# carlobaldassi/gimp-lqr-plugin

Measured on AMD Instinct MI355X. Metric: Mseams*pixels/sec on 4K RGBA, higher is better.
Workload: dtype f32; 1 GPU; batch4k: 64 x 3840x2160 RGBA per GPU, resize to 3640x2160 (200 vertical seams each), side-switch 2; images_per_gpu=64, width=3840, height=2160, new_width=3640, new_height=2160, parallelism=images sharded i mod N, no data-path collective, streams_per_gpu=1

## Files before the change

gimp-lqr-plugin_amd/csrc/k_backtrack.hip:

```cpp
#include "lqr_common.h"
#include "lqr_kernels.h"

__device__ __forceinline__ int row_argmin(const gf32 *mrow, int w, int lr, float *s_val, int *s_idx)
{
    const int tid = threadIdx.x;
    const float INF = __int_as_float(0x7f800000);
    float bv = INF;
    int bi = -1;
    for (int base = 0; base < w; base += 16 * VPATH_THREADS) {
        f32x4 v[4];
#pragma unroll
        for (int i = 0; i < 4; i++) {
            const int x = base + 4 * (tid + VPATH_THREADS * i);
            if (x + 3 < w) v[i] = *(const GLOBAL_AS f32x4 *) (mrow + x);
            else { v[i] = (f32x4) {INF, INF, INF, INF}; for (int j = 0; j < 4; j++) if (x + j < w) v[i][j] = mrow[x + j]; }
        }
#pragma unroll
        for (int i = 0; i < 4; i++)
#pragma unroll
            for (int j = 0; j < 4; j++) {
                const int x = base + 4 * (tid + VPATH_THREADS * i) + j;
                const float f = v[i][j];
                if (x < w && (f < bv || (f == bv && lr))) { bv = f; bi = x; }
            }
    }
    auto better = [&](float v2, int i2, float v1, int i1) {
        if (i2 < 0) return false;
        if (i1 < 0) return true;
        if (v2 < v1) return true;
        if (v2 > v1) return false;
        return lr ? (i2 > i1) : (i2 < i1);
    };
    for (int o = 32; o > 0; o >>= 1) {
        const float v2 = __shfl_xor(bv, o);
        const int i2 = __shfl_xor(bi, o);
        if (better(v2, i2, bv, bi)) { bv = v2; bi = i2; }
    }
    if ((tid & 63) == 0) { s_val[tid >> 6] = bv; s_idx[tid >> 6] = bi; }
    __syncthreads();
    bv = s_val[0]; bi = s_idx[0];
#pragma unroll
    for (int k = 1; k < VPATH_THREADS / 64; k++) if (better(s_val[k], s_idx[k], bv, bi)) { bv = s_val[k]; bi = s_idx[k]; }
    const float lim = 536870912.0f;
    const bool ok = (bi >= 0) && (bv < lim || (bv == lim && lr));
    return ok ? bi : -1;
}

__device__ unsigned long long g_moved_bytes;
__device__ __forceinline__ void publish_side(const GCarver &c, int org, int acc, int w, int h, int lane, int moved_unit)
{
    for (int o = 32; o > 0; o >>= 1) acc += __shfl_xor(acc, o);
    const long long all = (long long) h * (w - 1);
    const int side = (2ll * acc < all) ? 1 : 0;
    if (lane == 0) {
        c.flags[FLAG_ORG_PREV] = org; c.flags[FLAG_SIDE] = side; c.flags[FLAG_ORG] = org + side;
        atomicAdd(&g_moved_bytes, (unsigned long long) (side ? (long long) acc : all - acc) * (unsigned long long) moved_unit);
    }
}
extern "C" int lqrhip_moved_bytes(unsigned long long *out, int reset)
{
    if (lqrhip_init() < 0) return -1;
    (void) hipDeviceSynchronize();
    if (hipMemcpyFromSymbol(out, HIP_SYMBOL(g_moved_bytes), sizeof(unsigned long long)) != hipSuccess) return -1;
    if (reset) { unsigned long long z = 0; (void) hipMemcpyToSymbol(HIP_SYMBOL(g_moved_bytes), &z, sizeof z); }
    return 0;
}

__global__ __launch_bounds__(VPATH_THREADS) void k_vpath(const DevCarver *cs, int w, int h, int stride, int lr, int delta,
                                                          int log_index, int moved_unit)
{
    const GCarver c = gview(cs[blockIdx.x]);
    const int org = c.flags[FLAG_ORG];
    __shared__ float s_val[VPATH_THREADS / 64];
    __shared__ int s_idx[VPATH_THREADS / 64];
    const int tid = threadIdx.x;

    const int xmin = row_argmin(c.m + (size_t) (h - 1) * stride, w, lr, s_val, s_idx);
    if (tid >= 64) return;
    int x = __builtin_amdgcn_readfirstlane(max(xmin, 0));

    const int lane = tid;
    gi32 *seam = c.seam_x;
    gi32 *logp = c.seam_log + (size_t) log_index * h;
    const int R = delta > 0 ? min(VP_ROWS, max(1, VP_ROWS / delta)) : VP_ROWS;
    uint32_t regs[2][VP_ROWS];
    auto window_base = [&](int cx) { return (cx - 126) & ~3; };
    auto load_chunk = [&](int b, int y_top, int xa) {
        const int xl = xa + 4 * lane;
        const bool ok = (xl >= 0) && (xl + 3 < stride);
#pragma unroll
        for (int r = 0; r < VP_ROWS; r++) {
            const int y = max(y_top - r, 0);
            regs[b][r] = ok ? *(const gu32 *) (c.least + (size_t) y * stride + xl) : 0u;
        }
    };
    int y_top = h - 1;
    int xa_cur = window_base(x);
    int acc = 0;
    if (y_top >= 1) load_chunk(0, y_top, xa_cur);
    while (y_top >= 1) {
#pragma unroll
        for (int b = 0; b < 2; b++) {
            if (y_top >= 1) {
                const int nrows = min(R, y_top);
                const int xa_next = window_base(x);
                if (y_top - nrows >= 1) load_chunk(b ^ 1, y_top - nrows, xa_next);
                int path = 0;
#pragma unroll
                for (int r = 0; r < VP_ROWS; r++) {
                    if (r < nrows) {
                        path = (lane == r) ? x : path;
                        const int o = x - xa_cur;
                        const uint32_t dw = (uint32_t) __builtin_amdgcn_readlane((int) regs[b][r], o >> 2);
                        int d = (int) (int8_t) (dw >> (8 * (o & 3)));
                        d = (d == LEAST_INVALID) ? 0 : d;
                        x += d;
                    }
                }
                if (lane < nrows) { seam[y_top - lane] = path; logp[y_top - lane] = path; acc += path; }
                xa_cur = xa_next;
                y_top -= nrows;
            }
        }
    }
    if (lane == 0) { seam[0] = x; logp[0] = x; acc += x; }
    publish_side(c, org, acc, w, h, lane, moved_unit);
}

constexpr int vp1_rows(int delta) { return delta == 1 ? 28 : delta == 2 ? 12 : delta == 3 ? 8 : 4; }
#define VP1_AHEAD 3
template <int r>
__device__ __forceinline__ void vp1_step(const int e, int &o, int &path)
{
    asm volatile("v_writelane_b32 %0, %1, %2" : "+v"(path) : "s"(o), "n"(r));
    o += __builtin_amdgcn_readlane(e, o);
}
template <int N, int... Rs>
__device__ __forceinline__ void vp1_chase(const int (&e)[N], int &o, int &path, std::integer_sequence<int, Rs...>)
{
    (vp1_step<Rs>(e[Rs], o, path), ...);
}

template <int DELTA>
__global__ __launch_bounds__(VPATH_THREADS) void k_vpath1(const DevCarver *cs, int w, int h, int stride, int lr, int log_index, int moved_unit)
{
    const GCarver c = gview(cs[blockIdx.x]);
    const int org = c.flags[FLAG_ORG];
    __shared__ float s_val[VPATH_THREADS / 64];
    __shared__ int s_idx[VPATH_THREADS / 64];
    constexpr int VP1_ROWS = vp1_rows(DELTA);
    __shared__ __attribute__((aligned(16))) int8_t s_win[VP1_ROWS * 256];
    const int tid = threadIdx.x;

    const int xmin = row_argmin(c.m + (size_t) (h - 1) * stride, w, lr, s_val, s_idx);
    if (tid >= 64) return;
    int x = __builtin_amdgcn_readfirstlane(max(xmin, 0));

    const int lane = tid;
    gi32 *seam = c.seam_x;
    gi32 *logp = c.seam_log + (size_t) log_index * h;
    constexpr int R = VP1_ROWS, NB = VP1_AHEAD + 1, RL = VP1_ROWS / 4;
    static_assert(VP1_ROWS % 4 == 0 && VP1_ROWS * DELTA <= 28 && VP1_AHEAD * VP1_ROWS * DELTA + 32 <= 120, "window margin");
    u32x4 regs[NB][RL];
    int xa[NB];
    auto window_base = [&](int cx) { return (cx - 120) & ~15; };
    auto load_chunk = [&](int b, int y_top, int cx) {
        const int base = window_base(cx);
        xa[b] = base;
        const int voff = min(max(base + 16 * (lane & 15), 0), stride - 16);
        const int rsub = (lane >> 4) * stride;
#pragma unroll
        for (int q = 0; q < RL; q++) {
            const int row = max((y_top - 4 * q) * stride - rsub, stride);
            regs[b][q] = *(const GLOBAL_AS u32x4 *) (c.least + (unsigned) (row + voff));
        }
    };
    int acc = 0;
    auto run_chunk = [&](int b, int y_top) {
        const int relbase = x - 32 - xa[b];
        int e[R];
#pragma unroll
        for (int q = 0; q < RL; q++) *(u32x4 *) (s_win + q * 1024 + lane * 16) = regs[b][q];
        __builtin_amdgcn_wave_barrier();
#pragma unroll
        for (int r = 0; r < R; r++) e[r] = s_win[r * 256 + relbase + lane];
        int e2[R / 2];
#pragma unroll
        for (int k = 0; k < R / 2; k++) e2[k] = e[2 * k] + __builtin_amdgcn_ds_bpermute((lane + e[2 * k]) << 2, e[2 * k + 1]);
        int o = 32, path = 0;
        vp1_chase<R / 2>(e2, o, path, std::make_integer_sequence<int, R / 2>{});
        const int odd = path + s_win[min(lane, R / 2 - 1) * 512 + relbase + path];
        __builtin_amdgcn_wave_barrier();
        const int pe = path + x - 32, po = odd + x - 32;
        const int nrows = min(R, y_top);
        if (2 * lane < nrows) { seam[y_top - 2 * lane] = pe; logp[y_top - 2 * lane] = pe; acc += pe; }
        if (2 * lane + 1 < nrows) { seam[y_top - 2 * lane - 1] = po; logp[y_top - 2 * lane - 1] = po; acc += po; }
        x = (nrows == R) ? x + o - 32 : __builtin_amdgcn_readlane((nrows & 1) ? po : pe, nrows >> 1);
    };
    int y_top = h - 1;
#pragma unroll
    for (int k = 0; k < VP1_AHEAD; k++) load_chunk(k, y_top - k * R, x);
    while (true) {
#pragma unroll
        for (int k = 0; k < NB; k++) {
            load_chunk((k + VP1_AHEAD) % NB, y_top - VP1_AHEAD * R, x);
            run_chunk(k, y_top);
            y_top -= R;
            if (y_top < 1) break;
        }
        if (y_top < 1) break;
    }
    if (lane == 0) { seam[0] = x; logp[0] = x; acc += x; }
    publish_side(c, org, acc, w, h, lane, moved_unit);
}


template <int DELTA>
__global__ __launch_bounds__(256) void k_vp_maps(const DevCarver *cs, int w, int h, int stride)
{
    constexpr int R = vp_chunk_rows(DELTA), RD = R * DELTA, WIN = 256 + 2 * RD, R4 = (R + 3) / 4;
    __shared__ __attribute__((aligned(4))) int8_t s_rows[R][WIN + 8];
    const GCarver c = gview(cs[blockIdx.z]);
    const int chunk = blockIdx.y, ytop = h - 1 - chunk * R, nrows = min(R, ytop);
    const int X0 = blockIdx.x * 256, base = X0 - RD, tid = threadIdx.x;
    constexpr int WD = (WIN + 3) / 4, NI = (R * WD + 255) / 256;
    uint32_t v[NI];
#pragma unroll
    for (int k = 0; k < NI; k++) {
        const int i = tid + 256 * k, r = i / WD, d = i - r * WD, col = base + 4 * d;
        v[k] = 0u;
        if (i >= nrows * WD) continue;
        if (col >= 0 && col + 3 < stride) v[k] = *(const gu32 *) (c.least + (size_t) (ytop - r) * stride + col);
        else for (int b = 0; b < 4; b++) if (col + b >= 0 && col + b < stride) v[k] |= (uint32_t) (uint8_t) c.least[(size_t) (ytop - r) * stride + col + b] << (8 * b);
    }
#pragma unroll
    for (int k = 0; k < NI; k++) {
        const int i = tid + 256 * k, r = i / WD, d = i - r * WD;
        if (i < nrows * WD) *(uint32_t *) &s_rows[r][4 * d] = v[k];
    }
    __syncthreads();
    const int x = X0 + tid;
    if (x >= w) return;
    int p = x - base;
    gu32 *path = (gu32 *) c.vp_path + (size_t) chunk * R4 * stride + x;
#pragma unroll
    for (int r4 = 0; r4 < R4; r4++) {
        uint32_t pk = 0u;
#pragma unroll
        for (int k = 0; k < 4; k++) {
            const int r = 4 * r4 + k;
            pk |= (uint32_t) (uint8_t) (int8_t) (p + base - x) << (8 * k);
            if (r < nrows) { const int d = s_rows[r < R ? r : 0][p]; p += (d == LEAST_INVALID) ? 0 : d; }
        }
        path[(size_t) r4 * stride] = pk;
    }
    c.vp_map[(size_t) chunk * stride + x] = (int8_t) (p + base - x);
}

template <int DELTA>
__global__ __launch_bounds__(VPATH_THREADS) void k_vp_solve(const DevCarver *cs, int w, int h, int stride, int lr, int log_index, int moved_unit)
{
    constexpr int R = vp_chunk_rows(DELTA), RD = R * DELTA, S = VP_STAGE, R4 = (R + 3) / 4;
    constexpr int CP = (2 * RD * S + 4 + 15 + 16) & ~15;
    const GCarver c = gview(cs[blockIdx.x]);
    const int org = c.flags[FLAG_ORG];
    __shared__ float s_val[VPATH_THREADS / 64];
    __shared__ int s_idx[VPATH_THREADS / 64];
    __shared__ __attribute__((aligned(16))) int8_t s_cone[S][CP];
    extern __shared__ int s_xs[];
    __shared__ int s_acc[VPATH_THREADS / 64];
    const int tid = threadIdx.x, lane = tid & 63;
    const int xmin = row_argmin(c.m + (size_t) (h - 1) * stride, w, lr, s_val, s_idx);
    const int nchunks = (h - 1 + R - 1) / R;
    int x = max(xmin, 0);
    for (int c0 = 0; c0 < nchunks; c0 += S) {
        const int ns = min(S, nchunks - c0);
        const int base = (x - RD * S) & ~3;
        constexpr int W16 = CP / 16, NI = (S * W16 + VPATH_THREADS - 1) / VPATH_THREADS;
        u32x4 v[NI];
#pragma unroll
        for (int k = 0; k < NI; k++) {
            const int i = tid + k * VPATH_THREADS, j = i / W16, d = i - j * W16, col = base + 16 * d;
            v[k] = (u32x4) {0u, 0u, 0u, 0u};
            if (i >= ns * W16 || col + 15 < x - RD * (j + 1) || col > x + RD * (j + 1)) continue;
            const gi8 *src = c.vp_map + (size_t) (c0 + j) * stride + col;
            if (col >= 0 && col + 15 < stride) v[k] = *(const GLOBAL_AS u32x4 *) src;
            else {
                uint32_t q4[4] = {0u, 0u, 0u, 0u};
                for (int b = 0; b < 16; b++) if (col + b >= 0 && col + b < stride) q4[b >> 2] |= (uint32_t) (uint8_t) src[b] << (8 * (b & 3));
                v[k] = (u32x4) {q4[0], q4[1], q4[2], q4[3]};
            }
        }
#pragma unroll
        for (int k = 0; k < NI; k++) {
// ... 40 lines not shown
```

gimp-lqr-plugin_amd/csrc/k_carve.hip:

```cpp
#include "lqr_common.h"
#include "lqr_kernels.h"


#ifndef CG
#define CG 4
#endif
#define CGPX (CG * 256)
struct G32 { u32x4 a[CG]; uint32_t edge; };
struct G8 { uint32_t a[CG]; uint32_t edge; };

__device__ __forceinline__ void ld_left_u32(const gu32 *row, int base, int pend, int lane, G32 &g)
{
#pragma unroll
    for (int u = 0; u < CG; u++) {
        const int x = base + u * 256 + lane * 4;
        g.a[u] = (x <= pend) ? __builtin_nontemporal_load((const GLOBAL_AS u32x4 *) (row + x)) : (u32x4) {0u, 0u, 0u, 0u};
    }
    g.edge = (lane == 63 && base + CGPX <= pend) ? row[base + CGPX] : 0u;
}
__device__ __forceinline__ void st_left_u32(gu32 *row, int base, int pv, int pend, int lane, const G32 &g)
{
#pragma unroll
    for (int u = 0; u < CG; u++) {
        const int x = base + u * 256 + lane * 4;
        const uint32_t first_next = (u < CG - 1) ? (uint32_t) __builtin_amdgcn_readlane((int) g.a[u < CG - 1 ? u + 1 : CG - 1].x, 0) : 0u;
        const uint32_t lane63 = (u < CG - 1) ? first_next : g.edge;
        const uint32_t nx = (uint32_t) __builtin_amdgcn_update_dpp((int) lane63, (int) g.a[u].x, DPP_WAVE_SHL1, 0xf, 0xf, false);
        if (x < pend) {
            u32x4 o;
            o.x = (x >= pv) ? g.a[u].y : g.a[u].x;
            o.y = (x + 1 >= pv) ? g.a[u].z : g.a[u].y;
            o.z = (x + 2 >= pv) ? g.a[u].w : g.a[u].z;
            o.w = (x + 3 >= pv) ? nx : g.a[u].w;
            __builtin_nontemporal_store(o, (GLOBAL_AS u32x4 *) (row + x));
        }
    }
}

__device__ __forceinline__ void ld_right_u32(const gu32 *row, int gbase, int pbeg, int pv, int lane, G32 &g)
{
#pragma unroll
    for (int u = 0; u < CG; u++) {
        const int x = gbase + u * 256 + lane * 4;
        g.a[u] = (x + 3 >= pbeg && x <= pv) ? __builtin_nontemporal_load((const GLOBAL_AS u32x4 *) (row + x)) : (u32x4) {0u, 0u, 0u, 0u};
    }
    g.edge = (lane == 0 && gbase - 1 >= pbeg) ? row[gbase - 1] : 0u;
}
__device__ __forceinline__ void st_right_u32(gu32 *row, int gbase, int pbeg, int pv, int lane, const G32 &g)
{
#pragma unroll
    for (int u = 0; u < CG; u++) {
        const int x = gbase + u * 256 + lane * 4;
        const uint32_t last_prev = (u > 0) ? (uint32_t) __builtin_amdgcn_readlane((int) g.a[u > 0 ? u - 1 : 0].w, 63) : 0u;
        const uint32_t lane0 = (u > 0) ? last_prev : g.edge;
        const uint32_t pw = (uint32_t) __builtin_amdgcn_update_dpp((int) lane0, (int) g.a[u].w, DPP_WAVE_SHR1, 0xf, 0xf, false);
        if (x <= pv && x + 3 > pbeg) {
            u32x4 o;
            o.x = (x > pbeg && x <= pv) ? pw : g.a[u].x;
            o.y = (x + 1 > pbeg && x + 1 <= pv) ? g.a[u].x : g.a[u].y;
            o.z = (x + 2 > pbeg && x + 2 <= pv) ? g.a[u].y : g.a[u].z;
            o.w = (x + 3 > pbeg && x + 3 <= pv) ? g.a[u].z : g.a[u].w;
            __builtin_nontemporal_store(o, (GLOBAL_AS u32x4 *) (row + x));
        }
    }
}

__device__ __forceinline__ void st_left_en(gu32 *row, int base, int x0, int pend, int lane, const G32 &g)
{
#pragma unroll
    for (int u = 0; u < CG; u++) {
        const int x = base + u * 256 + lane * 4;
        const uint32_t first_next = (u < CG - 1) ? (uint32_t) __builtin_amdgcn_readlane((int) g.a[u < CG - 1 ? u + 1 : CG - 1].x, 0) : 0u;
        const uint32_t lane63 = (u < CG - 1) ? first_next : g.edge;
        const uint32_t nx = (uint32_t) __builtin_amdgcn_update_dpp((int) lane63, (int) g.a[u].x, DPP_WAVE_SHL1, 0xf, 0xf, false);
        if (x >= x0 && x < pend) __builtin_nontemporal_store((u32x4) {g.a[u].y, g.a[u].z, g.a[u].w, nx}, (GLOBAL_AS u32x4 *) (row + x));
    }
}
__device__ __forceinline__ void st_right_en(gu32 *row, int gbase, int x0, int x1, int lane, const G32 &g)
{
#pragma unroll
    for (int u = 0; u < CG; u++) {
        const int x = gbase + u * 256 + lane * 4;
        const uint32_t last_prev = (u > 0) ? (uint32_t) __builtin_amdgcn_readlane((int) g.a[u > 0 ? u - 1 : 0].w, 63) : 0u;
        const uint32_t lane0 = (u > 0) ? last_prev : g.edge;
// ... 27 lines not shown
        const int q = xo + dx;
        if (q == vprev) dx = LEAST_INVALID;
        else dx = q - (q > vprev ? 1 : 0) - xx;
    }
    return dx;
}

__device__ __forceinline__ void ld_left_8(const gu32 *row32, int base, int pend, int lane, G8 &g)
{
#pragma unroll
    for (int u = 0; u < CG; u++) {
        const int x = base + u * 256 + lane * 4;
        g.a[u] = (x <= pend) ? __builtin_nontemporal_load(row32 + (x >> 2)) : 0u;
    }
    g.edge = (lane == 63 && base + CGPX <= pend) ? row32[(base + CGPX) >> 2] : 0u;
}
__device__ __forceinline__ void st_left_8(gu32 *row32, int base, int org, int start, int v, int vprev, int y, int wnew, int lane, const G8 &g)
{
    const int pend = org + wnew;
#pragma unroll
    for (int u = 0; u < CG; u++) {
        const int x = base + u * 256 + lane * 4;
        const uint32_t first_next = (u < CG - 1) ? (uint32_t) __builtin_amdgcn_readlane((int) g.a[u < CG - 1 ? u + 1 : CG - 1], 0) : 0u;
        const uint32_t lane63 = (u < CG - 1) ? first_next : g.edge;
        const uint32_t nx = (uint32_t) __builtin_amdgcn_update_dpp((int) lane63, (int) g.a[u], DPP_WAVE_SHL1, 0xf, 0xf, false);
        if (x < pend) {
            const uint64_t both = ((uint64_t) nx << 32) | g.a[u];
            uint32_t o = 0;
#pragma unroll
            for (int j = 0; j < 4; j++) {
                const int xx = x + j - org;
                int dx;
                if (xx < start || xx >= wnew) {
                    dx = (int8_t) (g.a[u] >> (8 * j));
                } else {
                    const bool right = (xx >= v);
                    dx = rebase_dx((int8_t) (both >> (8 * (j + (right ? 1 : 0)))), xx, right ? xx + 1 : xx, vprev, y);
                }
                o |= (uint32_t) (uint8_t) (int8_t) dx << (8 * j);
            }
            __builtin_nontemporal_store(o, row32 + (x >> 2));
        }
    }
}

__device__ __forceinline__ void ld_right_8(const gu32 *row32, int gbase, int org, int ptop, int lane, G8 &g)
{
#pragma unroll
    for (int u = 0; u < CG; u++) {
        const int x = gbase + u * 256 + lane * 4;
        g.a[u] = (x + 3 >= org && x < ptop) ? __builtin_nontemporal_load(row32 + (x >> 2)) : 0u;
    }
    g.edge = (lane == 0 && gbase - 1 >= org) ? row32[(gbase - 4) >> 2] : 0u;
}
__device__ __forceinline__ void st_right_8(gu32 *row32, int gbase, int org, int end_l, int v, int vprev, int y, int lane, const G8 &g)
{
    const int pfirst = org + 1, ptop = org + 1 + end_l;
#pragma unroll
    for (int u = 0; u < CG; u++) {
        const int x = gbase + u * 256 + lane * 4;
        const uint32_t last_prev = (u > 0) ? (uint32_t) __builtin_amdgcn_readlane((int) g.a[u > 0 ? u - 1 : 0], 63) : 0u;
        const uint32_t lane0 = (u > 0) ? last_prev : g.edge;
        const uint32_t pd = (uint32_t) __builtin_amdgcn_update_dpp((int) lane0, (int) g.a[u], DPP_WAVE_SHR1, 0xf, 0xf, false);
        if (x < ptop && x + 3 >= pfirst) {
            const uint64_t both = ((uint64_t) g.a[u] << 8) | (pd >> 24);
            uint32_t o = 0;
#pragma unroll
            for (int j = 0; j < 4; j++) {
                const int xx = x + j - pfirst;
                int dx;
                if (xx < 0 || xx >= end_l) {
                    dx = (int8_t) (g.a[u] >> (8 * j));
                } else {
                    const bool right = (xx >= v);
                    dx = rebase_dx((int8_t) (both >> (8 * (j + (right ? 1 : 0)))), xx, right ? xx + 1 : xx, vprev, y);
                }
                o |= (uint32_t) (uint8_t) (int8_t) dx << (8 * j);
            }
            __builtin_nontemporal_store(o, row32 + (x >> 2));
        }
    }
}

template <bool BESIDE>
__device__ __forceinline__ void carve_row(const GCarver &c, int org, int side, int y, int w, int stride, int delta, int move_dp, int lane, int h = 0, int radius = 0)
{
    const int wnew = w - 1;
    int pa = 0x7fffffff, pb = -1;
    if (BESIDE) {
        int xmin, xmax;
        nrg_interval(c.seam_x, y, h, wnew, radius, xmin, xmax);
        if (xmin <= xmax) { pa = org + side + xmin; pb = org + side + xmax; }
    }
    const int v = c.seam_x[y];
    const size_t ro = (size_t) y * stride;
    const int vprev = y > 0 ? c.seam_x[y - 1] : 0;
    gu32 *en = (gu32 *) (c.en + ro), *mm = (gu32 *) (c.m + ro), *l32 = (gu32 *) (c.least + ro);
    gu32 *rg = c.rig ? (gu32 *) (c.rig + ro) : (gu32 *) nullptr;
    if (side == 0) {
        const int pv = org + v, pend = org + wnew;
        int start = (y > 0) ? min(v, vprev - delta) : v;
        if (start < 0) start = 0;
        int x0 = 0, fq = -1;
        uint32_t fval = 0;
        if (BESIDE) fq = en_fix_left(en, pv, pend, pb, lane, x0, fval);
        for (int base = (org + (move_dp ? start : v)) & ~3; base < pend; base += CGPX) {
            G32 E, M;
            G8 L;
            ld_left_u32(en, base, pend, lane, E);
            if (move_dp) { ld_left_u32(mm, base, pend, lane, M); ld_left_8(l32, base, pend, lane, L); }
            if (BESIDE) st_left_en(en, base, x0, pend, lane, E); else st_left_u32(en, base, pv, pend, lane, E);
            if (move_dp) { st_left_u32(mm, base, pv, pend, lane, M); st_left_8(l32, base, org, start, v, vprev, y, wnew, lane, L); }
        }
        if (BESIDE && fq >= 0) __builtin_nontemporal_store(fval, en + fq);
        if (rg)
            for (int base = pv & ~3; base < pend; base += CGPX) { G32 R; ld_left_u32(rg, base, pend, lane, R); st_left_u32(rg, base, pv, pend, lane, R); }
    } else {
        const int pv = org + v;
        const int end_l = (y > 0) ? min(wnew, max(v, vprev + delta)) : min(wnew, v);
        const int ptop = org + 1 + max(end_l, 0);
        const int top_u = (pv | 3) + 1;
        int x0 = 0, x1 = 0, fq = -1;
        uint32_t fval = 0;
        if (BESIDE) fq = en_fix_right(en, org, pv, pa, lane, x0, x1, fval);
        for (int top = move_dp ? max(top_u, (ptop + 3) & ~3) : top_u; top > org + 1; top -= CGPX) {
            const int gbase = top - CGPX;
            G32 E, M;
            G8 L;
            ld_right_u32(en, gbase, org, pv, lane, E);
            if (move_dp) { ld_right_u32(mm, gbase, org, pv, lane, M); ld_right_8(l32, gbase, org, ptop, lane, L); }
            if (BESIDE) st_right_en(en, gbase, x0, x1, lane, E); else st_right_u32(en, gbase, org, pv, lane, E);
            if (move_dp) { st_right_u32(mm, gbase, org, pv, lane, M); st_right_8(l32, gbase, org, max(end_l, 0), v, vprev, y, lane, L); }
        }
        if (BESIDE && fq >= 0) __builtin_nontemporal_store(fval, en + fq);
        if (rg)
            for (int top = top_u; top > org + 1; top -= CGPX) { G32 R; ld_right_u32(rg, top - CGPX, org, pv, lane, R); st_right_u32(rg, top - CGPX, org, pv, lane, R); }
    }
}

__global__ __launch_bounds__(256) void k_carve(const DevCarver *cs, int w, int h, int stride, int delta, int move_dp)
{
    const GCarver c = gview_phys(cs[blockIdx.y]);
    const int org = c.flags[FLAG_ORG_PREV], side = c.flags[FLAG_SIDE];
    const int lane = threadIdx.x & 63;
    if (blockIdx.x == 0 && threadIdx.x == 0) c.flags[FLAG_OVF_ROW] = h;
    for (int y = blockIdx.x * 4 + (threadIdx.x >> 6); y < h; y += gridDim.x * 4) carve_row<false>(c, org, side, y, w, stride, delta, move_dp, lane);
}

template <int NRG>
__global__ __launch_bounds__(256) void k_carve_e(const DevCarver *cs, DpK p, int w, int h, int stride, int move_dp, int k, int epoch)
{
    constexpr int NT = 12;
    constexpr bool luma = (NRG >= 3);
    const GCarver c = gview_phys(cs[blockIdx.y]);
    const int org = c.flags[FLAG_ORG_PREV], side = c.flags[FLAG_SIDE];
    const int lane = threadIdx.x & 63, wv = threadIdx.x >> 6;
    __shared__ double s_n255[256];
    __shared__ double s_bt[4][3][NT];
    __shared__ float s_bb[4][3][NT];
    __shared__ int s_lo[4][3];
    fill_norm255(s_n255, threadIdx.x, 256);
    __syncthreads();
    if (blockIdx.x == 0 && threadIdx.x == 0) c.flags[FLAG_OVF_ROW] = h;
    const int wn = w - 1;
    gf32 *en = c.en + org + side;
    for (int y = blockIdx.x * 4 + wv; y < h; y += gridDim.x * 4) {
        carve_row<false>(c, org, side, y, w, stride, p.delta, move_dp, lane);
        if (wn <= 1) continue;
        const int g = lane / NT, i = lane - g * NT, t = y - 1 + g;
        const bool samp = lane < 3 * NT && t >= 0 && t < h;
        int lo = 0, r = -1, pos = 0;
        if (samp) {
            int xmin, xmax;
            nrg_interval(c.seam_x, t, h, wn, p.radius, xmin, xmax);
            int l = xmin - 1; r = xmax + 1;
            if (t > 0) { int a, b; nrg_interval(c.seam_x, t - 1, h, wn, p.radius, a, b); if (b >= a) { l = min(l, a); r = max(r, b); } }
            if (t < h - 1) { int a, b; nrg_interval(c.seam_x, t + 1, h, wn, p.radius, a, b); if (b >= a) { l = min(l, a); r = max(r, b); } }
            lo = max(l, 0);
            pos = lo + i;
            const gi32 *lg = c.seam_log + t;
            for (int j = k; j >= epoch; j -= EU_LOGB) {
                int v[EU_LOGB];
#pragma unroll
                for (int u = 0; u < EU_LOGB; u++) v[u] = lg[(size_t) max(j - u, epoch) * h];
#pragma unroll
                for (int u = 0; u < EU_LOGB; u++) { const int vu = (j - u >= epoch) ? v[u] : 0x7fffffff; pos += (vu <= pos) ? 1 : 0; }
            }
            const int wf = wn + (k - epoch) + 1;
            const bool ok = (lo + i <= min(r, wn - 1)) && pos < wf;
            const size_t o = (size_t) t * stride + (ok ? pos : 0);
            s_bt[wv][g][i] = ok ? px_bright(c.pix[o], p.ch, luma, Norm255Lut{s_n255}) : 0.0;
            s_bb[wv][g][i] = (ok && c.bias) ? c.bias[o] : 0.0f;
            if (i == 0) s_lo[wv][g] = lo;
        }
        __builtin_amdgcn_wave_barrier();
        int xmin, xmax;
        nrg_interval(c.seam_x, y, h, wn, p.radius, xmin, xmax);
        const int x = xmin + lane;
        if (x <= xmax) {
            float e = grad_energy_f<NRG>([&](int xx, int yy) { const int gg = yy - y + 1; return s_bt[wv][gg][xx - s_lo[wv][gg]]; }, x, y, wn, h);
            if (c.bias) e = __fadd_rn(e, __fdiv_rn(s_bb[wv][1][x - s_lo[wv][1]], (float) p.w_start));
            asm volatile("s_waitcnt vmcnt(0)" ::: "memory");
            en[(size_t) y * stride + x] = e;
        }
        __builtin_amdgcn_wave_barrier();
    }
}

template <int NRG>
__global__ __launch_bounds__(256) void k_carve_u(const DevCarver *cs, DpK p, int w, int h, int stride, int move_dp, int k, int epoch, int n)
{
    const int eblk = (h + EU_ROWS - 1) / EU_ROWS, ne = n * eblk;
    if ((int) blockIdx.x < ne) {
        const int img = blockIdx.x / eblk, blk = blockIdx.x - img * eblk;
        PixRead<false> rd;
        rd.setup(threadIdx.x, 256);
        if (threadIdx.x >= 64) return;
        const GCarver c = gview(cs[img]);
        emap_update_block<NRG, 12, false, true>(c, rd, p, w - 1, h, stride, k, epoch, blk, threadIdx.x);
        return;
    }
    const int rblk = (h + 3) / 4, cb = blockIdx.x - ne, img = cb / rblk, rb = cb - img * rblk;
    const GCarver c = gview_phys(cs[img]);
    const int org = c.flags[FLAG_ORG_PREV], side = c.flags[FLAG_SIDE];
    if (rb == 0 && threadIdx.x == 0) c.flags[FLAG_OVF_ROW] = h;
    const int y = rb * 4 + (threadIdx.x >> 6);
    if (y < h) carve_row<true>(c, org, side, y, w, stride, p.delta, move_dp, threadIdx.x & 63, h, p.radius);
}

#define INST(N) template __global__ void k_carve_u<N>(const DevCarver *, DpK, int, int, int, int, int, int, int);
K_CARVE_U_FORMS(INST)
#undef INST
#define INST(N) template __global__ void k_carve_e<N>(const DevCarver *, DpK, int, int, int, int, int, int);
K_CARVE_E_FORMS(INST)
#undef INST
```

gimp-lqr-plugin_amd/csrc/lqr_common.h:

```cpp
#pragma once
#include <hip/hip_runtime.h>
#include <utility>
#include <type_traits>
#include <stdint.h>
#include <stdio.h>
#include <stdlib.h>
#include <string.h>
#include <string>
#include <vector>
#include <algorithm>
#include <map>
#include <unistd.h>

#include "../../include/lqr_hip.h"
#include "lqr_plan.h"

#define LEAST_INVALID (-128)
#define FLAG_OVF_ROW 0
#define FLAG_ORG 3
#define FLAG_ORG_PREV 4
#define FLAG_SIDE 5
#define FLAG_COUNT 8
#define FLAG_WORDS 64
#define VPATH_THREADS 256
// ... 104 lines not shown
struct Norm255Div { __device__ __forceinline__ double operator()(uint32_t v) const { return norm255(v); } };
struct Norm255Lut {
    const double *t;
    __device__ __forceinline__ double operator()(uint32_t v) const { return t[v]; }
};
__device__ __forceinline__ void fill_norm255(double *t, int tid, int nthreads)
{
    for (int v = tid; v < 256; v += nthreads) t[v] = norm255((uint32_t) v);
}
template <class N255>
__device__ __forceinline__ double px_bright(uint32_t p, int ch, bool luma, N255 norm255)
{
    double b;
    uint32_t c0 = p & 0xffu, c1 = (p >> 8) & 0xffu, c2 = (p >> 16) & 0xffu, c3 = p >> 24;
    if (ch <= 2) {
        b = norm255(c0);
        if (ch == 2) b = __dmul_rn(b, norm255(c1));
    } else {
        double r = norm255(c0), g = norm255(c1), bl = norm255(c2);
        if (luma)
            b = __dadd_rn(__dadd_rn(__dmul_rn(0.2126, r), __dmul_rn(0.7152, g)), __dmul_rn(0.0722, bl));
        else
            b = __ddiv_rn(__dadd_rn(__dadd_rn(r, g), bl), 3.0);
        if (ch == 4) b = __dmul_rn(b, norm255(c3));
    }
    return b;
}

template <int NRG, class BF>
__device__ __forceinline__ float grad_energy_f(BF B, int x, int y, int w, int h)
{
    if (NRG == 6) return 0.0f;
    constexpr int kind = NRG % 3;
    double gx, gy = 0.0;
    if (kind != 2) {
        if (h == 1) gy = 0.0;
        else if (y == 0) gy = __dsub_rn(B(x, 1), B(x, 0));
        else if (y < h - 1) gy = __dmul_rn(__dsub_rn(B(x, y + 1), B(x, y - 1)), 0.5);
        else gy = __dsub_rn(B(x, y), B(x, y - 1));
    }
    if (w == 1) gx = 0.0;
    else if (x == 0) gx = __dsub_rn(B(1, y), B(0, y));
    else if (x < w - 1) gx = __dmul_rn(__dsub_rn(B(x + 1, y), B(x - 1, y)), 0.5);
    else gx = __dsub_rn(B(x, y), B(x - 1, y));
    double g;
    if (kind == 0) g = __dsqrt_rn(__dadd_rn(__dmul_rn(gx, gx), __dmul_rn(gy, gy)));
    else if (kind == 1) g = __dmul_rn(__dadd_rn(fabs(gx), fabs(gy)), 0.5);
    else g = fabs(gx);
    return __double2float_rn(g);
}

template <int NRG, class N255>
__device__ __forceinline__ float grad_energy(const gu32 *pix, int stride, int x, int y, int w, int h, int ch, N255 n255)
{
    constexpr bool luma = (NRG >= 3);
    return grad_energy_f<NRG>([&](int xx, int yy) { return px_bright(pix[(size_t) yy * stride + xx], ch, luma, n255); }, x, y, w, h);
}

template <int NRG, class N255>
__device__ __forceinline__ float energy_at(const GCarver &c, const DpK &p, int stride, int x, int y, int w, int h, N255 n255)
{
    float e = grad_energy<NRG>(c.pix, stride, x, y, w, h, p.ch, n255);
    if (c.bias) e = __fadd_rn(e, __fdiv_rn(c.bias[(size_t) y * stride + x], (float) p.w_start));
    return e;
}

#define DPP_WAVE_SHL1 0x130
#define DPP_WAVE_SHR1 0x138

__device__ __forceinline__ int block_rank_256(bool flag, int *s_wave, int &total)
{
    const int lane = threadIdx.x & 63, wv = threadIdx.x >> 6;
    unsigned long long bal = __ballot(flag);
    int r = __popcll(bal & ((1ull << lane) - 1ull));
    __syncthreads();
    if (lane == 0) s_wave[wv] = __popcll(bal);
    __syncthreads();
    int off = 0;
    total = 0;
    for (int i = 0; i < 4; i++) { int t = s_wave[i]; if (i < wv) off += t; total += t; }
    return r + off;
}

__device__ __forceinline__ void nrg_interval(const gi32 *seam, int y, int h, int w, int radius, int &xmin, int &xmax)
{
    int y1a = max(y - radius, 0), y1b = min(y + radius, h - 1);
    int lo = seam[y], hi = seam[y] - 1;
    for (int y1 = y1a; y1 <= y1b; y1++) {
        int x = seam[y1];
        lo = min(lo, x - radius);
        hi = max(hi, x + radius - 1);
    }
    xmin = max(0, lo);
    xmax = min(w - 1, hi);
}

template <bool LR, bool RIG, bool UPDATE, bool MASK>
__device__ __forceinline__ void dp_row4(const float (&mp)[4], const float left, const float right, const f32x4 e, const f32x4 mo, const uint32_t lo4,
                                        const bool (&in)[4], const float rig_l, const float rig_r, float (&mc)[4], uint32_t &lnew, bool (&ch)[4])
{
    typedef float f32x2 __attribute__((ext_vector_type(2)));
    const float INF = __int_as_float(0x7f800000);
    float best[4];
    uint32_t sel[4];
#pragma unroll
    for (int k = 0; k < 4; k++) {
        float l = (k == 0) ? left : mp[k > 0 ? k - 1 : 0];
        const float cc = mp[k];
        float rr = (k == 3) ? right : mp[k < 3 ? k + 1 : 0];
        if (RIG) { l = __fadd_rn(l, rig_l); rr = __fadd_rn(rr, rig_r); }
        best[k] = fminf(fminf(l, cc), rr);
        const uint32_t minus = 0xffu << (8 * k), plus = 0x01u << (8 * k);
        if (LR) { sel[k] = (cc == best[k]) ? 0u : minus; sel[k] = (rr == best[k]) ? plus : sel[k]; }
        else { sel[k] = (cc == best[k]) ? 0u : plus; sel[k] = (l == best[k]) ? minus : sel[k]; }
    }
    const f32x2 nm01 = (f32x2) {e[0], e[1]} + (f32x2) {best[0], best[1]}, nm23 = (f32x2) {e[2], e[3]} + (f32x2) {best[2], best[3]};
    const float nm[4] = {nm01[0], nm01[1], nm23[0], nm23[1]};
    lnew = (sel[0] | sel[1]) | (sel[2] | sel[3]);
    if (UPDATE) {
        const uint32_t diff = lo4 ^ lnew;
        const f32x2 d01 = (f32x2) {mo[0], mo[1]} - nm01, d23 = (f32x2) {mo[2], mo[3]} - nm23;
        const float dd[4] = {d01[0], d01[1], d23[0], d23[1]};
#pragma unroll
        for (int k = 0; k < 4; k++) {
            float d = fabsf(dd[k]);
            d = ((diff >> (8 * k)) & 0xffu) ? INF : d;
            ch[k] = d > 1e-5f;
            const float v = ch[k] ? nm[k] : mo[k];
            mc[k] = (!MASK || in[k]) ? v : INF;
        }
    } else {
#pragma unroll
        for (int k = 0; k < 4; k++) mc[k] = (!MASK || in[k]) ? nm[k] : INF;
    }
}

template <int PX, bool LR, bool RIG, bool UPDATE, bool MASK>
__device__ __forceinline__ void dp_row(const float (&mp)[PX], const float left, const float right, const float (&e)[PX], const float (&mo)[PX],
                                       const uint32_t lo, const bool (&in)[PX], const float rig_l, const float rig_r, float (&mc)[PX],
                                       uint32_t &lnew, bool (&ch)[PX])
{
    typedef float f32x2 __attribute__((ext_vector_type(2)));
    static_assert(PX % 2 == 0, "pixel pairs");
    const float INF = __int_as_float(0x7f800000);
    float best[PX], nm[PX], dd[PX];
    uint32_t sel[PX];
#pragma unroll
    for (int k = 0; k < PX; k++) {
        float l = (k == 0) ? left : mp[k > 0 ? k - 1 : 0];
        const float cc = mp[k];
        float rr = (k == PX - 1) ? right : mp[k < PX - 1 ? k + 1 : 0];
        if (RIG) { l = __fadd_rn(l, rig_l); rr = __fadd_rn(rr, rig_r); }
        best[k] = fminf(fminf(l, cc), rr);
        const uint32_t minus = 0xffu << (8 * k), plus = 0x01u << (8 * k);
        if (LR) { sel[k] = (cc == best[k]) ? 0u : minus; sel[k] = (rr == best[k]) ? plus : sel[k]; }
        else { sel[k] = (cc == best[k]) ? 0u : plus; sel[k] = (l == best[k]) ? minus : sel[k]; }
    }
#pragma unroll
    for (int j = 0; j < PX / 2; j++) {
        const f32x2 s2 = (f32x2) {e[2 * j], e[2 * j + 1]} + (f32x2) {best[2 * j], best[2 * j + 1]};
        nm[2 * j] = s2[0]; nm[2 * j + 1] = s2[1];
        if (UPDATE) {
            const f32x2 d2 = (f32x2) {mo[2 * j], mo[2 * j + 1]} - s2;
            dd[2 * j] = d2[0]; dd[2 * j + 1] = d2[1];
        }
    }
    lnew = sel[0];
#pragma unroll
    for (int k = 1; k < PX; k++) lnew |= sel[k];
    const uint32_t diff = lo ^ lnew;
#pragma unroll
    for (int k = 0; k < PX; k++) {
        float v = nm[k];
        if (UPDATE) {
            float d = fabsf(dd[k]);
            d = ((diff >> (8 * k)) & 0xffu) ? INF : d;
            ch[k] = d > 1e-5f;
// ... 97 lines not shown
```

gimp-lqr-plugin_amd/csrc/lqr_kernels.h:

```cpp
#pragma once
#include "lqr_common.h"
#include "lqr_pixel.h"


template <class FORM> __global__ void k_wk_init(const DevCarver *cs, int w, int h, int stride, typename FORM::Arg a);
template <class FORM> __global__ __launch_bounds__(256) void k_wk_init_visible(const DevCarver *cs, int w0, int h, int stride, typename FORM::Arg a);
#define K_EMAP_FORMS(X) X(0, false) X(1, false) X(2, false) X(3, false) X(4, false) X(5, false) X(6, false) X(0, true) X(1, true) X(2, true) X(6, true)
#define K_EMAP_UPDATE_NT_FORMS(X, ...) X(12, __VA_ARGS__) X(36, __VA_ARGS__) X(68, __VA_ARGS__)
template <int NRG, bool VALUE> __global__ void k_emap_full(const DevCarver *cs, DpK p, int w, int h, int stride);
#define K_WK_INIT_EMAP_FORMS(X) X(0) X(1) X(2) X(3) X(4) X(5) X(6)
template <int NRG> __global__ __launch_bounds__(256) void k_wk_init_emap(const DevCarver *cs, DpK p, int w, int h, int stride);
__global__ void k_mask_add(float *plane, int w0, const uint8_t *mask, int channels, int mw, int x0, int y0, int x1, int y1,
                           int nx, int ny, int transposed, int is_rig, int bias_factor);
template <int NRG, int EU_NT, bool VALUE> __global__ __launch_bounds__(64) void k_emap_update(const DevCarver *cs, DpK p, int w, int h, int stride, int k, int epoch);
template <bool VALUE> __global__ __launch_bounds__(256) void k_frozen_catchup(const DevCarver *cs, int from, int to, int w_from, int h, int stride);

__global__ __launch_bounds__(VPATH_THREADS) void k_vpath(const DevCarver *cs, int w, int h, int stride, int lr, int delta, int log_index, int moved_unit);
#define K_VPATH1_FORMS(X) X(1) X(2) X(3) X(4) X(5) X(6) X(7)
#define K_VP_FORMS(X) K_VPATH1_FORMS(X) X(8) X(9) X(10)
template <int DELTA> __global__ __launch_bounds__(VPATH_THREADS) void k_vpath1(const DevCarver *cs, int w, int h, int stride, int lr, int log_index, int moved_unit);

template <int DELTA> __global__ __launch_bounds__(256) void k_vp_maps(const DevCarver *cs, int w, int h, int stride);
template <int DELTA> __global__ __launch_bounds__(VPATH_THREADS) void k_vp_solve(const DevCarver *cs, int w, int h, int stride, int lr, int log_index, int moved_unit);

__global__ __launch_bounds__(256) void k_carve(const DevCarver *cs, int w, int h, int stride, int delta, int move_dp);
#define K_CARVE_E_FORMS(X) X(0) X(1) X(2) X(3) X(4) X(5) X(6)
template <int NRG> __global__ __launch_bounds__(256) void k_carve_e(const DevCarver *cs, DpK p, int w, int h, int stride, int move_dp, int k, int epoch);
#define K_CARVE_U_FORMS(X) X(0) X(1) X(2) X(3) X(4) X(5) X(6)
template <int NRG> __global__ __launch_bounds__(256) void k_carve_u(const DevCarver *cs, DpK p, int w, int h, int stride, int move_dp, int k, int epoch, int n);

#define K_DP_SWEEP_PXT_FORMS(X) X(1) X(2) X(4) X(8) X(16)
#define K_LR_RIG_FORMS(X) X(false, false) X(false, true) X(true, false) X(true, true)
template <int PXT, bool UPDATE, int NTH = DP_THREADS> __global__ __launch_bounds__(NTH) void k_dp_sweep(const DevCarver *cs, DpK p, int w, int h, int stride, int lr);
__global__ __launch_bounds__(64) void k_band_update(const DevCarver *cs, DpK p, int w, int h, int stride, int lr);
template <int PXL, int NW, int R, bool LR, bool RIG> __global__ __launch_bounds__(64 * NW) void k_band_update_mw(const DevCarver *cs, DpK p, int w, int h, int stride);
template <int NW, bool LR, bool RIG> __global__ __launch_bounds__(128 * NW) void k_band_update_tw(const DevCarver *cs, DpK p, int w, int h, int stride, int *dev_err);

template <bool LR, bool RIG> __global__ __launch_bounds__(64) void k_dp_tile(const DevCarver *cs, DpK p, int w, int h, int stride, int y0);
#define K_DP_TILE_P_FORMS_D(X, LR, UPD, D) X(GENERAL, 2, LR, false, UPD, D, false, 16) X(GENERAL, 2, LR, true, UPD, D, false, 16) X(GENERAL, 2, LR, true, UPD, D, true, 16)
#define K_DP_TILE_P_FORMS_W(X, LR, UPD, D) X(GENERAL, 2, LR, true, UPD, D, false, 16) X(GENERAL, 2, LR, true, UPD, D, true, 16)
#define K_DP_TILE_P_FORMS_LR(X, LR, UPD) \
    X(PX4, 4, LR, false, UPD, 1, false, 16) X(PX4, 4, LR, true, UPD, 1, false, 16) X(PLAIN, 2, LR, false, UPD, 1, false, 16) X(PLAIN, 2, LR, true, UPD, 1, false, 16) \
    X(GENERAL, 2, LR, true, UPD, 1, true, 16) K_DP_TILE_P_FORMS_D(X, LR, UPD, 2) K_DP_TILE_P_FORMS_D(X, LR, UPD, 3) K_DP_TILE_P_FORMS_D(X, LR, UPD, 4) \
    K_DP_TILE_P_FORMS_W(X, LR, UPD, 5) K_DP_TILE_P_FORMS_W(X, LR, UPD, 6) K_DP_TILE_P_FORMS_W(X, LR, UPD, 7) K_DP_TILE_P_FORMS_W(X, LR, UPD, 8) K_DP_TILE_P_FORMS_W(X, LR, UPD, 9) K_DP_TILE_P_FORMS_W(X, LR, UPD, 10)
#define K_DP_TILE_P_FORMS_24(X, UPD) X(PLAIN, 2, false, false, UPD, 1, false, 24) X(PLAIN, 2, false, true, UPD, 1, false, 24) X(PLAIN, 2, true, false, UPD, 1, false, 24) X(PLAIN, 2, true, true, UPD, 1, false, 24)
#define K_DP_TILE_P_FORMS(X) K_DP_TILE_P_FORMS_LR(X, false, false) K_DP_TILE_P_FORMS_LR(X, false, true) K_DP_TILE_P_FORMS_LR(X, true, false) K_DP_TILE_P_FORMS_LR(X, true, true) \
    K_DP_TILE_P_FORMS_24(X, false) K_DP_TILE_P_FORMS_24(X, true)
template <int PX, bool LR, bool RIG, bool UPDATE, int DELTA = 1, bool RIGM = false, int HLN = 16>
__global__ __launch_bounds__(64 * DPP_W) void k_dp_tile_p(DevCarver *cs, DpK p, int w, int h, int stride, unsigned long long *exch, int epoch, int *dev_err);

#define K_BAND_LEVELS_FORMS_D(X, LR, D) X(LR, false, D, false) X(LR, true, D, false) X(LR, true, D, true)
#define K_BAND_LEVELS_FORMS_W(X, LR, D) X(LR, true, D, false) X(LR, true, D, true)
#define K_BAND_LEVELS_FORMS_LR(X, LR) K_BAND_LEVELS_FORMS_D(X, LR, 1) K_BAND_LEVELS_FORMS_D(X, LR, 2) K_BAND_LEVELS_FORMS_D(X, LR, 3) K_BAND_LEVELS_FORMS_D(X, LR, 4) \
    K_BAND_LEVELS_FORMS_W(X, LR, 5) K_BAND_LEVELS_FORMS_W(X, LR, 6) K_BAND_LEVELS_FORMS_W(X, LR, 7) K_BAND_LEVELS_FORMS_W(X, LR, 8) K_BAND_LEVELS_FORMS_W(X, LR, 9) K_BAND_LEVELS_FORMS_W(X, LR, 10)
#define K_BAND_LEVELS_FORMS(X) K_BAND_LEVELS_FORMS_LR(X, false) K_BAND_LEVELS_FORMS_LR(X, true)
template <bool LR, bool RIG, int DELTA, bool RIGM>
__global__ __launch_bounds__(128) __attribute__((amdgpu_waves_per_eu(2, 2))) void k_band_levels(DevCarver *cs, DpK p, int w, int h, int stride, unsigned long long *exch, int epoch, int *dev_err, int P, int n_img);

__global__ __launch_bounds__(256) void k_vs_commit(const DevCarver *cs, int w0, int h0, int wc0, int n_seams, int first_level, int finish);
template <bool DEEP> __global__ __launch_bounds__(256) void k_inflate(const InflateDev *jobs, int w0, int w1, int l, int max_level, int *dev_err);
__global__ __launch_bounds__(256) void k_vmap_check(const int32_t *map, int len, int depth, int *dev_err);
#define VT_LINES 32
__global__ __launch_bounds__(256) void k_vmap_check_t(const int32_t *map, int32_t *out, int width, int height, int depth, int *dev_err);
__global__ __launch_bounds__(256) void k_seam_check(const DevCarver *cs, int h, int wc0, int n_seams, int delta, int *dev_err);
__global__ __launch_bounds__(256) void k_vs_rollback(const DevCarver *cs, size_t n, int first_level, int finish_level);
__global__ void k_inject(const DevCarver *cs, int what, int h, int w0, int log_index, int first_level);
template <bool DEEP> __global__ __launch_bounds__(256) void k_compact(const uint8_t *rgb, const int32_t *vs, const float *bias, const float *rig,
                                                  uint8_t *nrgb, float *nbias, float *nrig, int32_t *nvmap, int w0, int w, int ch, int level, int depth);
template <bool DEEP> __global__ __launch_bounds__(256) void k_compact_jobs(const InflateDev *jobs, int w0, int w, int level);
__global__ void k_transpose(const InflateDev *jobs, int w, int h);
__global__ void k_transpose_px(const InflateDev *jobs, int w, int h);
__global__ __launch_bounds__(256) void k_mask_line_max(const uint8_t *mask, int channels, int width, int a0, int b0, int line_len, int direction, int *out);

template <class T> __global__ __launch_bounds__(256) void k_mask_add_f(float *plane, int w0, const T *mask, int mw, int x0, int y0, int x1, int y1, int nx, int ny,
                                                                       int transposed, int is_rig, int bias_factor);
__global__ __launch_bounds__(256) void k_mask_scatter(float *plane, const int *index, const double *value, size_t n, int is_rig);
__global__ __launch_bounds__(256) void k_plane_transpose(const float *plane, float *out, int w0, int h0);

template <bool PIC> __global__ __launch_bounds__(256) void k_energy_range(const DevCarver *cs, int w, int h, int stride, float *partials);
__global__ __launch_bounds__(256) void k_energy_plane(const DevCarver *cs, int w, int h, int stride, int transposed, int normalised,
                                                      const float *partials, int n_partials, float *out);
#define K_ENERGY_OUT_FORMS_T(X, T) X(T, 0) X(T, 1) X(T, 2) X(T, 3)
#define K_ENERGY_OUT_FORMS(X) K_ENERGY_OUT_FORMS_T(X, 0) K_ENERGY_OUT_FORMS_T(X, 1) K_ENERGY_OUT_FORMS_T(X, 2) K_ENERGY_OUT_FORMS_T(X, 3) K_ENERGY_OUT_FORMS_T(X, 4) K_ENERGY_OUT_FORMS_T(X, 5) K_ENERGY_OUT_FORMS_T(X, 6)
template <int TYPE, int DEPTH> __global__ __launch_bounds__(256) void k_energy_out(const DevCarver *cs, int w, int h, int stride, int transposed,
                                                                                    const float *partials, int n_partials, uint8_t *out);
```

gimp-lqr-plugin_amd/csrc/lqr_pixel.h:

```cpp
#pragma once
#include "lqr_common.h"

typedef GLOBAL_AS double gf64;

template <bool VALUE> struct PixRead;
template <> struct PixRead<false> {
    typedef uint32_t T;
    const double *n255;
    __device__ __forceinline__ void setup(int tid, int nthreads)
    {
        __shared__ double s_n255[256];
        fill_norm255(s_n255, tid, nthreads);
        __syncthreads();
        n255 = s_n255;
    }
    __device__ __forceinline__ double operator()(const gu32 *pix, size_t o, int ch, bool luma) const { return px_bright(pix[o], ch, luma, Norm255Lut{n255}); }
};
template <> struct PixRead<true> {
    typedef double T;
    __device__ __forceinline__ void setup(int, int) {}
    __device__ __forceinline__ double operator()(const gu32 *pix, size_t o, int, bool) const { return ((const gf64 *) pix)[o]; }
};

template <int NRG, int EU_NT, bool VALUE, bool ONE_WAVE>
__device__ __forceinline__ void emap_update_block(const GCarver c, const PixRead<VALUE> rd, const DpK p, int w, int h, int stride, int k, int epoch, unsigned blk, int tid)
{
    __shared__ double bt[64][EU_NT];
    __shared__ float bb[64][EU_NT];
    __shared__ int slo[64];
    const int y = blk * EU_ROWS + tid - 1;
    const bool row_ok = (y >= 0 && y < h);
    constexpr bool luma = (NRG >= 3);
    int xmin = 0, xmax = -1, lo = 0;
    if (row_ok) {
        nrg_interval(c.seam_x, y, h, w, p.radius, xmin, xmax);
        int l = xmin - 1, r = xmax + 1;
        if (y > 0) { int a, b; nrg_interval(c.seam_x, y - 1, h, w, p.radius, a, b); if (b >= a) { l = min(l, a); r = max(r, b); } }
        if (y < h - 1) { int a, b; nrg_interval(c.seam_x, y + 1, h, w, p.radius, a, b); if (b >= a) { l = min(l, a); r = max(r, b); } }
        lo = max(l, 0);
        int pos[EU_NT];
#pragma unroll
        for (int i = 0; i < EU_NT; i++) pos[i] = lo + i;
        const gi32 *lg = c.seam_log + y;
        for (int j = k; j >= epoch; j -= EU_LOGB) {
            int v[EU_LOGB];
#pragma unroll
            for (int u = 0; u < EU_LOGB; u++) v[u] = lg[(size_t) max(j - u, epoch) * h];
#pragma unroll
            for (int u = 0; u < EU_LOGB; u++) {
                const int vu = (j - u >= epoch) ? v[u] : 0x7fffffff;
#pragma unroll
                for (int i = 0; i < EU_NT; i++) pos[i] += (vu <= pos[i]) ? 1 : 0;
            }
        }
        const int wf = w + (k - epoch) + 1;
#pragma unroll
        for (int i = 0; i < EU_NT; i++) {
            const bool ok = (lo + i <= min(r, w - 1)) && pos[i] < wf;
            const size_t o = (size_t) y * stride + (ok ? pos[i] : 0);
            bt[tid][i] = ok ? rd(c.pix, o, p.ch, luma) : 0.0;
            bb[tid][i] = (ok && c.bias) ? c.bias[o] : 0.0f;
        }
    }
    slo[tid] = lo;
    if (ONE_WAVE) __builtin_amdgcn_wave_barrier(); else __syncthreads();
    if (!row_ok || tid == 0 || tid == 63) return;
    for (int x = xmin; x <= xmax; x++) {
        float e = grad_energy_f<NRG>([&](int xx, int yy) { const int t = tid + (yy - y); return bt[t][xx - slo[t]]; }, x, y, w, h);
        if (c.bias) e = __fadd_rn(e, __fdiv_rn(bb[tid][x - lo], (float) p.w_start));
        c.en[(size_t) y * stride + x] = e;
    }
}

template <int DEPTH>
__device__ __forceinline__ double deep_norm(const gu8 *px, int k)
{
    if (DEPTH == 0) return norm255(px[k]);
    if (DEPTH == 1) return __ddiv_rn((double) ((const GLOBAL_AS uint16_t *) px)[k], 65535.0);
    if (DEPTH == 2) return (double) ((const GLOBAL_AS float *) px)[k];
    return ((const gf64 *) px)[k];
}
template <int DEPTH>
__device__ __forceinline__ double deep_value(const gu8 *px, const DeepRead &rd)
{
    double b;
    if (rd.mode == RD_GREY) {
        b = deep_norm<DEPTH>(px, 0);
    } else if (rd.mode == RD_CUSTOM) {
        const bool has_black = rd.black >= 0;
        const double kf = __dsub_rn(1.0, has_black ? deep_norm<DEPTH>(px, rd.black) : 0.0);
        double s = 0.0;
        for (int k = 0; k < rd.ch; k++)
            if (k != rd.alpha && k != rd.black) s = __dadd_rn(s, __dsub_rn(1.0, __dmul_rn(__dsub_rn(1.0, deep_norm<DEPTH>(px, k)), kf)));
        s = __ddiv_rn(s, (double) (rd.ch - (rd.alpha >= 0 ? 1 : 0) - (has_black ? 1 : 0)));
        b = has_black ? __dsub_rn(1.0, s) : s;
    } else {
        double r = deep_norm<DEPTH>(px, 0), g = deep_norm<DEPTH>(px, 1), bl = deep_norm<DEPTH>(px, 2);
        if (rd.mode != RD_RGB) {
            r = __dsub_rn(1.0, r); g = __dsub_rn(1.0, g); bl = __dsub_rn(1.0, bl);
            if (rd.mode == RD_CMYK) {
                const double kf = __dsub_rn(1.0, deep_norm<DEPTH>(px, 3));
                r = __dmul_rn(r, kf); g = __dmul_rn(g, kf); bl = __dmul_rn(bl, kf);
            }
        }
        if (rd.luma)
            b = __dadd_rn(__dadd_rn(__dmul_rn(0.2126, r), __dmul_rn(0.7152, g)), __dmul_rn(0.0722, bl));
        else
            b = __ddiv_rn(__dadd_rn(__dadd_rn(r, g), bl), 3.0);
    }
    if (rd.alpha >= 0) b = __dmul_rn(b, deep_norm<DEPTH>(px, rd.alpha));
    return b;
}
struct PixPacked {
    typedef uint32_t T;
    typedef int Arg;
    static __device__ __forceinline__ T form(const gu8 *rgb0, size_t i, int ch)
    {
        const gu8 *s = rgb0 + i * ch;
        uint32_t p = 0;
        if (ch == 4) p = *(const gu32 *) s;
        else for (int k = 0; k < ch; k++) p |= (uint32_t) s[k] << (8 * k);
        return p;
    }
};
template <int DEPTH> struct PixValue {
    typedef double T;
    typedef DeepRead Arg;
    static __device__ __forceinline__ T form(const gu8 *rgb0, size_t i, const DeepRead &rd)
    {
        constexpr int bpc = DEPTH == 0 ? 1 : DEPTH == 1 ? 2 : DEPTH == 2 ? 4 : 8;
// ... 45 lines not shown
```

gimp-lqr-plugin_amd/csrc/lqr_plan.h:

```cpp
#pragma once
#include <algorithm>
#include <stddef.h>
#include "../../include/lqr_hip.h"

#define DP_THREADS 1024
constexpr int dppx_px(int px) { return px == 3 ? 2 : px; }
constexpr int dppx_hl(int px) { return px == 3 ? 24 : 16; }
constexpr int dpp_halo(int px) { return dppx_hl(px) * dppx_px(px); }
constexpr int dpp_own(int px) { return 64 * dppx_px(px) - 2 * dpp_halo(px); }
constexpr int dpp_ex_tile(int px) { return px == 3 ? 2 * dpp_own(3) : 2 * 2 * dpp_halo(px); }
constexpr int dpp_rb(int px, int delta) { return delta >= 5 ? dpp_halo(2) / delta : delta >= 3 ? 8 : dpp_halo(px) / delta; }
constexpr int DPP_R = 16;
constexpr int DPP_W = 2;
static_assert(dpp_halo(2) % (2 * DPP_R) == 0 && dpp_halo(4) % (2 * DPP_R) == 0, "a block (halo / delta_x rows, delta_x <= 2) is a whole number of batches");
constexpr int DPP_BLK_BITS = 12;
#define DPT_ROWS 32
#define DPT_OWN 192
constexpr int LV_PMAX = 16;
constexpr int LV_MAX_TILES = 64;
constexpr int LV_MAX_LEVELS = 1020;
constexpr int lv_rows(int delta, bool rigm = false) { return delta == 1 ? (rigm ? 16 : 32) : delta == 2 ? 16 : delta <= 4 ? 8 : 32 / delta; }
constexpr int LQR_FAST_MAX_DELTA = 10;
constexpr int VP_REACH = 56;
constexpr int VP_STAGE = 20;
constexpr int vp_chunk_rows(int delta) { return VP_REACH / delta; }
constexpr int eu_samples(int delta_x) { return delta_x <= 2 ? 12 : delta_x <= 8 ? 36 : 68; }
#ifndef FROZEN_LAG_MAX
#define FROZEN_LAG_MAX 128
#endif
constexpr int frozen_lag(int images) { return images <= 4 ? FROZEN_LAG_MAX / 4 : FROZEN_LAG_MAX; }
constexpr bool lds_needs_attr(size_t bytes) { return bytes > 64 * 1024; }
constexpr int LV_AUTO_MIN = 7;

struct PlanKnobs {
    int vpath_mode = -1;
    int vpath_par_max = 3, vpath_min_rows = 1000;
    int sweep_threads = 256;
    int carve_fused = 4;
    int carve_beside = -1;
    int update_mode = -1;
    int band_levels = -1;
    int dpp_limit = -1;
    int dpp_px = 0;
    int sub_batches = 0;
    long long tiled_update_px = 8LL * 3840 * 2160;
};
struct PlanDevice {
    int wgs_plain = 0, wgs_general = 0, wgs_px4 = 0, wgs_levels = 0;
    int n_cu = 0, hw_queues = 0;
};
struct PlanBatch {
    int images = 1;
    bool shared = false;
    int shared_n = 1;
    bool spin = true;
    int wk_h = 0;
    bool value = false;
    bool rigmask = false;
    size_t group() const { return (size_t) images * (size_t) std::max(shared_n, 1); }
    bool rigm(bool use_rig) const { return use_rig && rigmask; }
};

struct DpPlan {
    int form = -1, px = 0, per = 0, threads = 0;
    bool general = false;
    size_t lds = 0;
};
struct StepPlan {
    int backtrack = 0;
    int vp_rows = 0, vp_chunks = 0;
    int carve = 0;
    bool energy_beside = false;
    bool catchup = false;
    int eu_nt = 0;
    bool full = false;
    int band = -1;
    int levels_P = 0;
    DpPlan dp;
};

static inline int plan_limit(const PlanKnobs &k, int bound) { return k.dpp_limit >= 0 ? std::min(k.dpp_limit, bound) : bound; }
constexpr int tiles_of(int w, int own) { return (w + own - 1) / own; }

static inline int plan_streams(const PlanKnobs &k, const PlanDevice &d, int n)
{
    const int nb = k.sub_batches ? k.sub_batches : d.hw_queues >= 8 ? (n >= 49 ? 4 : n >= 32 ? 2 : 1) : 1;
    return n >= 2 * nb ? nb : 1;
}

static inline int plan_persistent_px(const PlanKnobs &k, const PlanDevice &d, const PlanBatch &b, int w, bool general, int delta, int images)
{
    if (b.shared || !b.spin) return 0;
    const size_t n = (size_t) images;
    const int limit = plan_limit(k, general ? d.wgs_general : d.wgs_plain);
    const int maxblk = (1 << DPP_BLK_BITS) - 1;
    if (!general && delta == 1 && (k.dpp_px == 3 || k.dpp_px == 0) && b.wk_h <= maxblk * dpp_rb(3, 1) &&
        tiles_of(w, dpp_own(3)) * n <= (size_t) std::min(limit, k.dpp_px == 3 ? limit : d.n_cu)) return 3;
    if ((general || (k.dpp_px != 4 && k.dpp_px != 3)) && b.wk_h <= maxblk * dpp_rb(2, delta) && tiles_of(w, dpp_own(2)) * n <= (size_t) limit) return 2;
    if (!general && k.dpp_px != 2 && k.dpp_px != 3 && b.wk_h <= maxblk * dpp_halo(4) && tiles_of(w, dpp_own(4)) * n <= (size_t) plan_limit(k, d.wgs_px4)) return 4;
    return 0;
}
static inline DpPlan plan_persistent(int px, bool general, int per)
{
    DpPlan p;
    p.form = general ? LQRHIP_CENSUS_TILE_P_GENERAL : px == 3 ? LQRHIP_CENSUS_TILE_P_G3 : px == 2 ? LQRHIP_CENSUS_TILE_P_G2 : LQRHIP_CENSUS_TILE_P_G4;
    p.px = px; p.general = general; p.per = per;
    return p;
}

static inline DpPlan plan_sweep(const PlanKnobs &k, int w, bool update)
{
    DpPlan p;
    p.form = update ? LQRHIP_CENSUS_SWEEP_UPDATE : LQRHIP_CENSUS_SWEEP_FULL;
    p.threads = (update && k.sweep_threads == 256 && w <= 16 * 256) ? 256 : DP_THREADS;
    for (p.px = 1; p.px <= 16 && p.px * p.threads < w;) p.px *= 2;
    if (p.px > 16) p.px = 0;
    p.lds = (size_t) 2 * ((w + 3) & ~3) * sizeof(float);
    return p;
}

static inline DpPlan plan_full_dp(const PlanKnobs &k, const PlanDevice &d, const PlanBatch &b, int w, int delta, bool use_rig)
{
    const bool general = delta != 1 || b.rigm(use_rig);
    if (delta >= 1 && delta <= LQR_FAST_MAX_DELTA) {
        int per = b.images, px;
        while (!(px = plan_persistent_px(k, d, b, w, general, delta, per)) && general && per > 1) per = (per + 1) / 2;
        if (px) return plan_persistent(px, general, per);
        if (!general) { DpPlan p; p.form = LQRHIP_CENSUS_DP_TILE; return p; }
    }
    return plan_sweep(k, w, false);
}

static inline bool levels_auto(const PlanKnobs &k, int delta, size_t group, bool plain)
{
    return k.update_mode < 0 && delta <= 4 && group >= 8 && (group <= 64 || !plain);
}
static inline int plan_levels_P(const PlanKnobs &k, const PlanDevice &d, const PlanBatch &b, int w, int h, int delta)
{
    if (!b.spin || k.band_levels == 0 || delta < 1 || delta > LQR_FAST_MAX_DELTA || tiles_of(h, lv_rows(delta, true)) > LV_MAX_LEVELS || tiles_of(w, 64) > LV_MAX_TILES) return 0;
    const int per_batch = plan_limit(k, d.wgs_levels) / std::max(b.shared_n, 1);
    const int want = k.band_levels > 0 ? k.band_levels : std::max(LV_AUTO_MIN, std::min(12, (int) ((b.shared ? 384 : 2 * d.n_cu) / std::max<size_t>(b.group(), 1))));
    const int P = std::min({LV_PMAX, per_batch / std::max(b.images, 1), want});
    return P >= (k.band_levels > 0 ? 1 : LV_AUTO_MIN) ? P : 0;
}
static inline int plan_general_batch_limit(const PlanKnobs &k, const PlanDevice &d, int w, int delta)
{
    const int tiled = plan_limit(k, d.wgs_general) / tiles_of(w, dpp_own(2));
    const int lv = plan_limit(k, d.wgs_levels) / LV_AUTO_MIN;
    return levels_auto(k, delta, (size_t) std::max(lv, 0), false) && k.band_levels != 0 && tiles_of(w, 64) <= LV_MAX_TILES ? std::max(tiled, lv) : tiled;
}

constexpr int CARVE_BESIDE_MIN = 8;
static inline bool plan_carve_beside(const PlanKnobs &k, const PlanBatch &b, int delta, int wnew)
{
    if (k.carve_beside == 0 || delta > 2 || b.value || wnew <= 1) return false;
    return k.carve_beside > 0 || (!b.shared && b.group() >= (size_t) CARVE_BESIDE_MIN);
}

static inline StepPlan plan_seam_step(const PlanKnobs &k, const PlanDevice &d, const PlanBatch &b, int delta, bool use_rig, int w, int h, bool full_rebuild, int lag)
{
    StepPlan s;
    const int wnew = w - 1, mode = k.update_mode;
    const bool fast_delta = delta >= 1 && delta <= LQR_FAST_MAX_DELTA, general = delta != 1 || b.rigm(use_rig);
    if (fast_delta && h >= 2 && k.vpath_mode != 0 && (k.vpath_mode == 1 || delta >= 5 || (b.group() <= (size_t) k.vpath_par_max && h >= k.vpath_min_rows))) {
        s.backtrack = LQRHIP_CENSUS_VP_PARALLEL;
        s.vp_rows = vp_chunk_rows(delta);
        s.vp_chunks = tiles_of(h - 1, s.vp_rows);
    } else s.backtrack = delta >= 1 && delta <= 7 ? LQRHIP_CENSUS_VPATH1 : LQRHIP_CENSUS_VPATH;
    s.carve = delta <= 2 && b.group() <= (size_t) k.carve_fused && wnew > 1 && !b.value ? LQRHIP_CENSUS_CARVE_E : LQRHIP_CENSUS_CARVE;
    s.energy_beside = s.carve == LQRHIP_CENSUS_CARVE && plan_carve_beside(k, b, delta, wnew);
    s.catchup = lag > frozen_lag(b.images);
    s.eu_nt = eu_samples(delta);
    if (wnew <= 1) return s;
    if (full_rebuild) {
        s.full = true;
        s.dp = plan_full_dp(k, d, b, wnew, delta, use_rig);
        return s;
    }
    const bool plain = !general && mode != 3;
    const bool tiled = (plain ? (mode < 0 ? (long long) b.images * w * h <= k.tiled_update_px : mode == 1) : (fast_delta && mode != 0 && mode != 2 && mode != 3)) &&
                       plan_persistent_px(k, d, b, w, general, delta, b.images) != 0;
    if (fast_delta && mode != 3 && (mode == 5 || levels_auto(k, delta, b.group(), plain))) s.levels_P = plan_levels_P(k, d, b, wnew, h, delta);
    if (s.levels_P > 0) s.band = LQRHIP_CENSUS_BAND_LEVELS;
    else if (tiled) {
        s.dp = plan_persistent(plan_persistent_px(k, d, b, wnew, general, delta, b.images), general, b.images);
        return s;
    } else if (plain && (size_t) h * sizeof(int) <= 60 * 1024) {
        s.band = mode != 2 && wnew <= 4200 && (size_t) 2 * h * sizeof(int) <= 64 * 1024 ? LQRHIP_CENSUS_BAND_TW : wnew > 4200 ? LQRHIP_CENSUS_BAND_MW16 : LQRHIP_CENSUS_BAND_MW8;
    } else s.band = LQRHIP_CENSUS_BAND_GENERIC;
    s.dp = plan_sweep(k, wnew, true);
    return s;
}
```

gimp-lqr-plugin_amd/csrc/lqr_shim.hip:

```cpp
#include "lqr_common.h"
#include "lqr_kernels.h"
#include "lqr_own.h"
#include "lqr_pool.h"
#include "lqr_stage.h"
#include <memory>
#include <dirent.h>

static thread_local std::string g_err;
static int g_device = -1;

static int *g_dev_err_host = nullptr;
static int *g_dev_err = nullptr;

#define HIPCK_VOID(expr) do { hipError_t e__ = (expr); if (e__ != hipSuccess) { g_err = std::string(#expr) + ": " + hipGetErrorString(e__); (void) hipGetLastError(); } } while (0)
#define HIPCK(expr)                                                                   \
    do {                                                                              \
        hipError_t e__ = (expr);                                                      \
        if (e__ != hipSuccess) {                                                      \
            g_err = std::string(#expr) + ": " + hipGetErrorString(e__);               \
            (void) hipGetLastError();                                                 \
            return (e__ == hipErrorOutOfMemory) ? LQRHIP_ENOMEM : LQRHIP_EHIP;        \
        }                                                                             \
    } while (0)

// ... 7 lines not shown
    DevBuf<int8_t> least, least2;
    DevBuf<int32_t> seam_x, seam_log, flags;
    DevBuf<int8_t> vp_map, vp_path;
};
}
struct __attribute__((visibility("hidden"))) LqrHipCarver {
    int ch = 0;
    int depth = 0;
    int luma = 0;
    int mode = RD_RGB, alpha = -1, black = -1;
    int pix_deep = 0;
    int w0 = 0, h0 = 0;
    DevBuf<uint8_t> rgb0;
    DevBuf<int32_t> vs;
    DevBuf<float> bias0, rig0;
    int active = 0;
    int stride = 0, wk_h = 0;
    WorkingPlanes wk;
    int log_cap = 0, log_h = 0;
    int frozen_epoch = 0;
    int owed_to = 0, owed_w = 0, owed_h = 0;
    LqrHipCarver *root = nullptr;
    std::vector<LqrHipCarver *> aux;
    LqrHipBatch *batch = nullptr;
};

static inline size_t px_bytes(const LqrHipCarver *c) { return (size_t) c->ch << (c->depth == 0 ? 0 : c->depth == 1 ? 1 : c->depth == 2 ? 2 : 3); }
static inline int32_t *vs_of(const LqrHipCarver *c) { return (c->root ? c->root : c)->vs; }

namespace {
struct PlaneJob {
    LqrHipCarver *c;
    DevBuf<uint8_t> nrgb;
    DevBuf<float> nbias, nrig;
};
}
struct PlaneJobs {
    std::vector<PlaneJob> jobs;
    std::vector<DevBuf<int32_t>> new_vs;
    std::vector<InflateDev> dev;
    DevBuf<InflateDev> d_dev;
    size_t n_narrow = 0;
    int add(LqrHipCarver *c, const int32_t *vs_old, int32_t *nvs, size_t n1)
    {
        jobs.push_back(PlaneJob{c, {}, {}, {}});
        PlaneJob &j = jobs.back();
        int rc = j.nrgb.alloc(n1 * px_bytes(c), "&j.nrgb");
        if (!rc && c->bias0) rc = j.nbias.alloc(n1, "&j.nbias");
        if (!rc && c->rig0) rc = j.nrig.alloc(n1, "&j.nrig");
        if (rc) return rc;
        dev.push_back(InflateDev{c->rgb0, vs_old, c->bias0, c->rig0, j.nrgb, nvs, j.nbias, j.nrig, (int) px_bytes(c), c->depth});
        return 0;
    }
    int stage(hipStream_t s, bool by_width)
    {
        n_narrow = std::stable_partition(dev.begin(), dev.end(), [&](const InflateDev &d) { return d.ch <= 4 && (by_width || d.depth == 0); }) - dev.begin();
        int rc = d_dev.alloc(dev.size(), "&d_dev");
        if (rc) return rc;
        HIPCK(hipMemcpyAsync(d_dev, dev.data(), dev.size() * sizeof(InflateDev), hipMemcpyHostToDevice, s));
        return 0;
    }
    size_t n_wide() const { return dev.size() - n_narrow; }
    const InflateDev *d_wide() const { return d_dev + n_narrow; }
};
static void commit(PlaneJobs &pj)
{
    for (auto &j : pj.jobs) {
        j.c->rgb0 = std::move(j.nrgb);
        if (j.nbias) j.c->bias0 = std::move(j.nbias);
        if (j.nrig) j.c->rig0 = std::move(j.nrig);
    }
}

struct PendingInflate { PlaneJobs pj; int kind = 0 , w1 = 0, h1 = 0; };

struct LqrHipBatch {
    std::vector<LqrHipCarver *> cs;
    DevCarver *d_desc = nullptr;
    size_t desc_cap = 0;
    hipStream_t stream = nullptr;
    DevBuf<unsigned long long> exch;
    int exch_ntiles = 0, exch_n = 0, exch_px = 0;
    int tile_epoch = 0;
    bool dirty = true;
    int shared_n = 1;
    bool shared = false;
    bool safe = false;
    std::unique_ptr<PendingInflate> pending_inflate;
};
static bool g_no_spin = false;

struct ProfRec {
    std::vector<std::pair<hipEvent_t, hipEvent_t>> ev;
    double bytes = 0;
};
static int g_prof = 0;
static std::map<std::string, ProfRec> g_profrec;
static hipStream_t g_stream0 = nullptr;
static unsigned long long g_census[LQRHIP_CENSUS_SLOTS];
#define CENSUS(slot) (g_census[(slot)]++)
extern "C" int lqrhip_launch_census(unsigned long long *out, int n, int reset)
{
    if (out && n > 0) memcpy(out, g_census, (size_t) std::min(n, (int) LQRHIP_CENSUS_SLOTS) * sizeof g_census[0]);
    if (reset) memset(g_census, 0, sizeof g_census);
    return LQRHIP_CENSUS_SLOTS;
}

extern "C" const char *lqrhip_last_error(void) { return g_err.c_str(); }

static void dpp_resident_workgroups(int dev)
{
    hipDeviceProp_t prop;
    if (hipGetDeviceProperties(&prop, dev) != hipSuccess || prop.multiProcessorCount <= 0) return;
    enum { PX4, PLAIN, GENERAL, LEVELS, N_CLASSES };
    int per_cu[N_CLASSES] = {1 << 20, 1 << 20, 1 << 20, 1 << 20};
    auto q = [&](int cls, auto kern, int threads) {
        int n = 0;
        if (hipOccupancyMaxActiveBlocksPerMultiprocessor(&n, kern, threads, 0) != hipSuccess) { (void) hipGetLastError(); n = 0; }
        per_cu[cls] = std::min(per_cu[cls], n);
    };
#define QUERY(CLASS, ...) q(CLASS, k_dp_tile_p<__VA_ARGS__>, 64 * DPP_W);
    K_DP_TILE_P_FORMS(QUERY)
#undef QUERY
#define QUERY(...) q(LEVELS, k_band_levels<__VA_ARGS__>, 128);
    K_BAND_LEVELS_FORMS(QUERY)
#undef QUERY
    auto bound = [&](int blocks) { return std::max(0, blocks - 1) * prop.multiProcessorCount; };
    g_dev.n_cu = prop.multiProcessorCount;
    g_dev.wgs_px4 = bound(per_cu[PX4]);
    g_dev.wgs_plain = bound(std::min(per_cu[PX4], per_cu[PLAIN]));
    g_dev.wgs_general = bound(per_cu[GENERAL]);
    g_dev.wgs_levels = bound(per_cu[LEVELS]);
}

static bool kfd_is_open(void)
{
    DIR *d = opendir("/proc/self/fd");
    if (!d) return true;
    bool open_ = false;
    while (struct dirent *e = readdir(d)) {
        if (e->d_name[0] == '.') continue;
        char path[64], link[64];
        snprintf(path, sizeof path, "/proc/self/fd/%s", e->d_name);
        const ssize_t n = readlink(path, link, sizeof link - 1);
        if (n <= 0) continue;
        link[n] = 0;
        if (strcmp(link, "/dev/kfd") == 0) { open_ = true; break; }
    }
    closedir(d);
    return open_;
}
__attribute__((constructor)) static void lqrhip_on_load(void)
{
    if (!kfd_is_open()) setenv("GPU_MAX_HW_QUEUES", "8", 0);
}

extern "C" int lqrhip_init(void)
{
    if (g_device >= 0) return g_device;
    int n = 0;
    if (hipGetDeviceCount(&n) != hipSuccess || n <= 0) {
        g_err = "no HIP device visible: the MI355X engine needs a gfx950 GPU (there is no CPU fallback)";
        (void) hipGetLastError();
        return LQRHIP_EHIP;
    }
    int dev = 0;
// ... 683 lines not shown
    HIPCK(hipGetLastError());
    return 0;
}

extern "C" int lqrhip_wk_init_emap(LqrHipBatch *b, const LqrHipDpParams *p, int w, int h)
{
    LqrHipCarver *c0 = b->cs[0];
    int rc;
    if (reads_value(c0) || w != c0->w0 || h != c0->h0) return (rc = lqrhip_wk_init(b, 0)) ? rc : lqrhip_emap_build(b, p, w, h);
    if ((rc = wk_init_prepare(b))) return rc;
    const dim3 grid((tiles_of(c0->stride, 4) + 255) / 256, h, (unsigned) b->cs.size());
    DpK k = make_dpk(p, c0->ch);
    const int nrg = nrg_index(p->nrg_func);
#define CASE(N) if (nrg == N) hipLaunchKernelGGL(k_wk_init_emap<N>, grid, dim3(256), 0, b->stream, b->d_desc, k, w, h, c0->stride); else
    K_WK_INIT_EMAP_FORMS(CASE) return no_form("k_wk_init_emap");
#undef CASE
    HIPCK(hipGetLastError());
    return 0;
}

extern "C" int lqrhip_energy_out(LqrHipBatch *b, int w, int h, int transposed, int form, int depth, int image_type, void *out, int on_device)
{
    static const int channels_of[7] = {3, 4, 1, 2, 3, 4, 5};
    if (b->cs.size() != 1 || !out || w < 1 || h < 1 || form < 0 || form > 2) { g_err = "energy read-out: one carver, a buffer, form 0 .. 2"; return LQRHIP_EARG; }
    if (form != 2) { depth = 2; image_type = 2; }
    if (depth < 0 || depth > 3 || image_type < 0 || image_type > 6) { g_err = "energy read-out: depth 0 .. 3, image type 0 .. 6"; return LQRHIP_EARG; }
    int rc;
    if ((rc = batch_upload(b))) return rc;
    LqrHipCarver *c0 = b->cs[0];
    if (!c0->wk.en) return LQRHIP_EARG;
    const size_t bytes = (size_t) w * h * channels_of[image_type] << depth;
    const int chunks = (w + EO_CHUNK - 1) / EO_CHUNK;
    const int n_partials = form ? (int) std::min((long long) EO_MAX_PARTIALS, (long long) h * chunks) : 0;
    Scratch tmp(b->stream);
    float *partials = form ? tmp.get<float>((size_t) 2 * n_partials, "&partials", rc) : nullptr;
    if (rc) return rc;
    uint8_t *staged = on_device ? nullptr : tmp.get<uint8_t>(bytes, "&staged", rc);
    if (rc) return rc;
    uint8_t *dst = on_device ? (uint8_t *) out : staged;
    {
        ProfScope prof("energy_out", b->stream, (double) w * h * sizeof(float) * (form ? 2 : 1) + (double) bytes);
        if (form == 1) hipLaunchKernelGGL(k_energy_range<false>, dim3(n_partials), dim3(256), 0, b->stream, b->d_desc, w, h, c0->stride, partials);
        if (form == 2) hipLaunchKernelGGL(k_energy_range<true>, dim3(n_partials), dim3(256), 0, b->stream, b->d_desc, w, h, c0->stride, partials);
        const int W = transposed ? h : w, H = transposed ? w : h;
        const dim3 grid((W + EO_TILE - 1) / EO_TILE, (H + EO_TILE - 1) / EO_TILE);
#define CASE(T, D) if (image_type == T && depth == D) hipLaunchKernelGGL((k_energy_out<T, D>), grid, dim3(256), 0, b->stream, b->d_desc, w, h, c0->stride, transposed, partials, n_partials, dst); else
        if (form != 2)
            hipLaunchKernelGGL(k_energy_plane, grid, dim3(256), 0, b->stream, b->d_desc, w, h, c0->stride, transposed, form, partials, n_partials, (float *) dst);
        else K_ENERGY_OUT_FORMS(CASE) return no_form("k_energy_out");
#undef CASE
    }
    hipError_t e = hipGetLastError();
    if (e == hipSuccess) e = hipStreamSynchronize(b->stream);
    if (e != hipSuccess) { g_err = std::string("energy read-out: ") + hipGetErrorString(e); (void) hipGetLastError(); return LQRHIP_EHIP; }
    if ((rc = check_dev_error())) return rc;
    if (!on_device && (rc = d2h_staged(out, staged, bytes))) return rc;
    tmp.done();
    return 0;
}

static int launch_dp_tiled(LqrHipBatch *b, const DpK &k, int w, int h, int lr)
{
    LqrHipCarver *c0 = b->cs[0];
    const dim3 grid((w + DPT_OWN - 1) / DPT_OWN, (unsigned) b->cs.size());
    for (int y0 = 0; y0 < h; y0 += DPT_ROWS) {
        CENSUS(LQRHIP_CENSUS_DP_TILE);
#define CASE(LRV, RIGV) if ((lr != 0) == LRV && (k.use_rig != 0) == RIGV) hipLaunchKernelGGL((k_dp_tile<LRV, RIGV>), grid, dim3(64), 0, b->stream, b->d_desc, k, w, h, c0->stride, y0); else
        K_LR_RIG_FORMS(CASE) return no_form("k_dp_tile");
#undef CASE
    }
    HIPCK(hipGetLastError());
    return 0;
}

extern "C" void lqrhip_set_vpath_mode(int mode, int par_max) { g_knobs.vpath_mode = mode; if (par_max > 0) g_knobs.vpath_par_max = par_max; }
extern "C" void lqrhip_set_sweep_threads(int n) { g_knobs.sweep_threads = n == 256 ? 256 : DP_THREADS; }
extern "C" void lqrhip_set_carve_fused(int max_images) { g_knobs.carve_fused = max_images == 1 ? 4 : max_images < 0 ? 0 : max_images; }
extern "C" void lqrhip_set_carve_beside(int mode) { g_knobs.carve_beside = mode < 0 ? -1 : mode ? 1 : 0; }
static unsigned long long g_carve_beside_launches;
extern "C" unsigned long long lqrhip_carve_beside_launches(int reset)
{
    const unsigned long long v = g_carve_beside_launches;
    if (reset) g_carve_beside_launches = 0;
    return v;
}
extern "C" void lqrhip_set_update_mode(int mode) { g_knobs.update_mode = mode; }
extern "C" void lqrhip_set_dp_persistent_px(int px) { g_knobs.dpp_px = (px == 2 || px == 3 || px == 4) ? px : 0; }
extern "C" void lqrhip_set_dp_persistent_limit(int workgroups) { g_knobs.dpp_limit = workgroups; }
extern "C" void lqrhip_set_band_levels(int slots) { g_knobs.band_levels = slots; }
static PlanBatch plan_batch(const LqrHipBatch *b)
{
    PlanBatch pb;
    pb.images = (int) b->cs.size(); pb.shared = b->shared; pb.shared_n = b->shared_n; pb.spin = !(b->safe || g_no_spin);
    pb.wk_h = b->cs[0]->wk_h; pb.value = reads_value(b->cs[0]);
    for (auto *c : b->cs) pb.rigmask |= c->wk.rig != nullptr;
    return pb;
}
extern "C" int lqrhip_general_batch_limit_delta(int w, int delta)
{
    return lqrhip_init() < 0 || w < 1 ? 0 : plan_general_batch_limit(g_knobs, g_dev, w, delta);
}
extern "C" int lqrhip_general_batch_limit(int w) { return lqrhip_general_batch_limit_delta(w, 2); }

static int exch_ensure(LqrHipBatch *b, size_t need_elems, int ntiles, int n, int layout)
{
    int rc;
    bool grew = false;
    if (b->exch.size() < need_elems) HIPCK(hipStreamSynchronize(b->stream));
    if ((rc = b->exch.ensure(need_elems, "&b->exch", &grew))) return rc;
    if (grew) b->exch_ntiles = 0;
    if (b->exch_ntiles != ntiles || b->exch_n != n || b->exch_px != layout) {
        HIPCK(hipMemsetAsync(b->exch, 0, need_elems * sizeof(unsigned long long), b->stream));
        b->exch_ntiles = ntiles; b->exch_n = n; b->exch_px = layout;
    }
    return 0;
}

struct DpForm { bool lr, rig; int delta; bool rigm; };
static inline DpForm dp_form(const DpK &k, int lr, bool rigm) { return DpForm{lr != 0, k.use_rig != 0 || k.delta >= 5, k.delta, rigm}; }

template <bool UPDATE>
static int launch_dp_persistent(LqrHipBatch *b, const DpK &k, const DpPlan &dp, bool rigm, int w, int h, int lr, int first, int count)
{
    LqrHipCarver *c0 = b->cs[0];
    const size_t n = (size_t) count;
    const int px = dp.px;
    const bool general = dp.general;
    if (!px || (UPDATE && n != b->cs.size())) return LQRHIP_EARG;
    const int ntiles = (w + dpp_own(px) - 1) / dpp_own(px);
    int rc;
    const size_t need_elems = 2 * ((size_t) ntiles * dpp_ex_tile(px) + 8) * n;
    if ((rc = exch_ensure(b, need_elems, ntiles, (int) n, px))) return rc;
    if (UPDATE) {
        bool grew = false;
        for (auto *c : b->cs) {
            if (c->wk.m2 && c->wk.least2) continue;
            if (!grew) { HIPCK(hipStreamSynchronize(b->stream)); grew = true; }
            const size_t pe = (size_t) c->stride * (c->wk_h + 1) + 1024;
            DevBuf<float> m2;
            DevBuf<int8_t> least2;
            if ((rc = m2.alloc(pe, "&c->m2")) || (rc = least2.alloc(pe, "&c->least2"))) return rc;
            hipError_t e = hipMemsetAsync(m2, 0, pe * sizeof(float), b->stream);
            if (e == hipSuccess) e = hipMemsetAsync(least2, 0, pe, b->stream);
            if (e != hipSuccess) { lqr_stream_wait(b->stream); HIPCK(e); }
            c->wk.m2 = std::move(m2); c->wk.least2 = std::move(least2);
        }
        if (grew) {
            b->dirty = true;
            if ((rc = batch_upload(b))) return rc;
        }
    }
    const int epoch = 1 + ((b->tile_epoch++) % ((1 << (31 - DPP_BLK_BITS)) - 2));
    const dim3 grid(ntiles, (unsigned) n);
    CENSUS(general ? LQRHIP_CENSUS_TILE_P_GENERAL : px == 3 ? LQRHIP_CENSUS_TILE_P_G3 : px == 2 ? LQRHIP_CENSUS_TILE_P_G2 : LQRHIP_CENSUS_TILE_P_G4);
    const DpForm f = dp_form(k, lr, rigm);
    const int px_lane = px == 4 ? 4 : 2, hln = px == 3 ? 24 : 16;
    const bool found = [&] {
#define CASE(CLASS, PX, LR, RIG, UPD, DELTA, RIGM, HLN)                                                                         \
        if constexpr (UPD == UPDATE)                                                                                            \
            if (px_lane == PX && f.lr == LR && f.rig == RIG && f.delta == DELTA && f.rigm == RIGM && hln == HLN) {              \
                hipLaunchKernelGGL((k_dp_tile_p<PX, LR, RIG, UPD, DELTA, RIGM, HLN>), grid, dim3(64 * DPP_W), 0, b->stream, b->d_desc + first, k, w, h, c0->stride, b->exch.get(), epoch, g_dev_err); \
                return true;                                                                                                    \
            }
        K_DP_TILE_P_FORMS(CASE)
#undef CASE
        return false;
// ... 100 lines not shown
    int rc;
    const int ntiles = (w + 63) / 64;
    const size_t need_elems = 2 * ((size_t) 4 * LV_PMAX + (size_t) 2 * ntiles * 64) * n;
    if ((rc = exch_ensure(b, need_elems, ntiles, (int) n, 103))) return rc;
    const int epoch = 1 + ((b->tile_epoch++) % ((1 << 22) - 2));
    const dim3 grid((unsigned) (8 * ((n + 7) / 8) * P));
    CENSUS(LQRHIP_CENSUS_BAND_LEVELS);
    const DpForm f = dp_form(k, lr, rigm);
#define CASE(LR, RIG, DELTA, RIGM) if (f.lr == LR && f.rig == RIG && f.delta == DELTA && f.rigm == RIGM) \
        hipLaunchKernelGGL((k_band_levels<LR, RIG, DELTA, RIGM>), grid, dim3(128), 0, b->stream, b->d_desc, k, w, h, c0->stride, b->exch.get(), epoch, g_dev_err, P, (int) n); else
    K_BAND_LEVELS_FORMS(CASE) return no_form("k_band_levels");
#undef CASE
    HIPCK(hipGetLastError());
    return 0;
}
static int seam_step_impl(LqrHipBatch *b, const LqrHipDpParams *p, int w, int h, int log_index, int leftright_pick,
                          int full_rebuild, int leftright_next);
static void inject_after_step(LqrHipBatch *b, int h, int log_index);
static void inject_after_commit(LqrHipBatch *b, int w0, int h0, int first_level);
extern "C" int lqrhip_seam_step(LqrHipBatch *b, const LqrHipDpParams *p, int w, int h, int log_index, int leftright_pick,
                                int full_rebuild, int leftright_next)
{
    const int rc = seam_step_impl(b, p, w, h, log_index, leftright_pick, full_rebuild, leftright_next);
    if (rc == 0) inject_after_step(b, h, log_index);
    static const char *dump = getenv("LQRHIP_DUMP");
    if (rc == 0 && dump) {
        static int call = 0;
        LqrHipCarver *c = b->cs[0];
        HIPCK(hipStreamSynchronize(b->stream));
        const size_t np = (size_t) c->stride * h;
        std::vector<int> hdr = {w, h, c->stride, log_index, FLAG_COUNT}, flags(FLAG_COUNT), seam(h);
        std::vector<float> m(np);
        std::vector<int8_t> least(np);
        HIPCK(hipMemcpy(flags.data(), c->wk.flags, FLAG_COUNT * sizeof(int), hipMemcpyDeviceToHost));
        HIPCK(hipMemcpy(seam.data(), c->wk.seam_x, (size_t) h * sizeof(int), hipMemcpyDeviceToHost));
        HIPCK(hipMemcpy(m.data(), c->wk.m, np * sizeof(float), hipMemcpyDeviceToHost));
        HIPCK(hipMemcpy(least.data(), c->wk.least, np, hipMemcpyDeviceToHost));
        char path[512];
        snprintf(path, sizeof path, "%s_%04d.bin", dump, call++);
        if (FILE *f = fopen(path, "wb")) {
            fwrite(hdr.data(), sizeof(int), hdr.size(), f); fwrite(flags.data(), sizeof(int), flags.size(), f);
            fwrite(seam.data(), sizeof(int), seam.size(), f); fwrite(m.data(), sizeof(float), np, f); fwrite(least.data(), 1, np, f);
            fclose(f);
        }
    }
    return rc;
}

static int seam_step_impl(LqrHipBatch *b, const LqrHipDpParams *p, int w, int h, int log_index, int leftright_pick,
                          int full_rebuild, int leftright_next)
{
    int rc;
    LqrHipCarver *c0 = b->cs[0];
    for (auto *c : b->cs)
        if (log_index >= c->log_cap || c->owed_to) return LQRHIP_EARG;
    if ((rc = batch_upload(b))) return rc;
    const unsigned n = (unsigned) b->cs.size();
    DpK k = make_dpk(p, c0->ch);
    const int stride = c0->stride;
    const int wnew = w - 1;
    const int move_dp = (wnew > 1 && !full_rebuild) ? 1 : 0;
    const PlanBatch pb = plan_batch(b);
    const StepPlan s = plan_seam_step(g_knobs, g_dev, pb, p->delta_x, p->use_rigidity != 0, w, h, full_rebuild != 0, log_index + 1 - c0->frozen_epoch);
    const bool rigm = pb.rigm(p->use_rigidity != 0);
    const int moved_unit = 2 * (4 + (move_dp ? 5 : 0) + (pb.rigmask ? 4 : 0));
    if (s.backtrack == LQRHIP_CENSUS_VP_PARALLEL) {
        const int nchunks = s.vp_chunks, R4 = (s.vp_rows + 3) / 4;
        const size_t need = (size_t) (nchunks + 1) * stride + 64, need_path = need * 4 * R4;
        bool grew = false;
        for (auto *c : b->cs) {
            WorkingPlanes &wp = c->wk;
            if (wp.vp_map.size() >= need && wp.vp_path.size() >= need_path) continue;
            if (!grew) { HIPCK(hipStreamSynchronize(b->stream)); grew = true; }
            wp.vp_map.reset(); wp.vp_path.reset();
            if ((rc = wp.vp_map.alloc(need, "&c->vp_map")) || (rc = wp.vp_path.alloc(need_path, "&c->vp_path"))) return rc;
        }
        if (grew) { b->dirty = true; if ((rc = batch_upload(b))) return rc; }
        ProfScope ps("vpath", b->stream, 0);
        CENSUS(LQRHIP_CENSUS_VP_PARALLEL);
        if (!with_listed(K_VP_FORMS, p->delta_x, [&](auto delta) {
                hipLaunchKernelGGL(k_vp_maps<delta>, dim3((w + 255) / 256, nchunks, n), dim3(256), 0, b->stream, b->d_desc, w, h, stride);
                hipLaunchKernelGGL(k_vp_solve<delta>, dim3(n), dim3(VPATH_THREADS), (size_t) (nchunks + 2) * sizeof(int), b->stream, b->d_desc, w, h, stride, leftright_pick, log_index, moved_unit);
            })) return no_form("k_vp_maps");
    } else {
        ProfScope ps("vpath", b->stream, 0);
        CENSUS(s.backtrack);
        if (!with_listed(K_VPATH1_FORMS, p->delta_x, [&](auto delta) {
                hipLaunchKernelGGL(k_vpath1<delta>, dim3(n), dim3(VPATH_THREADS), 0, b->stream, b->d_desc, w, h, stride, leftright_pick, log_index, moved_unit);
            }))
            hipLaunchKernelGGL(k_vpath, dim3(n), dim3(VPATH_THREADS), 0, b->stream, b->d_desc, w, h, stride, leftright_pick, p->delta_x,
                               log_index, moved_unit);
    }
    auto frozen_within_lag = [&]() -> int { return s.catchup ? frozen_catchup(b, log_index + 1, wnew, h) : 0; };
    const bool fuse_e = s.carve == LQRHIP_CENSUS_CARVE_E;
    if (fuse_e) {
        if ((rc = frozen_within_lag())) return rc;
        const int epoch = c0->frozen_epoch;
        ProfScope ps("carve", b->stream, 4.0 * (double) w * h * n);
        CENSUS(LQRHIP_CENSUS_CARVE_E);
        if (!with_listed(K_CARVE_E_FORMS, nrg_index(p->nrg_func), [&](auto nrg) {
                hipLaunchKernelGGL((k_carve_e<nrg>), dim3((h + 3) / 4, n), dim3(256), 0, b->stream, b->d_desc, k, w, h, stride, move_dp, log_index, epoch);
            })) return no_form("k_carve_e");
    } else if (s.energy_beside) {
        if ((rc = frozen_within_lag())) return rc;
        const int epoch = c0->frozen_epoch;
        ProfScope ps("carve", b->stream, 4.0 * (double) w * h * n);
        CENSUS(LQRHIP_CENSUS_CARVE);
        g_carve_beside_launches++;
        const unsigned grid = n * (unsigned) ((h + EU_ROWS - 1) / EU_ROWS) + n * (unsigned) ((h + 3) / 4);
        if (!with_listed(K_CARVE_U_FORMS, nrg_index(p->nrg_func), [&](auto nrg) {
                hipLaunchKernelGGL((k_carve_u<nrg>), dim3(grid), dim3(256), 0, b->stream, b->d_desc, k, w, h, stride, move_dp, log_index, epoch, (int) n);
            })) return no_form("k_carve_u");
    } else {
        ProfScope ps("carve", b->stream, 4.0 * (double) w * h * n);
        CENSUS(LQRHIP_CENSUS_CARVE);
        hipLaunchKernelGGL(k_carve, dim3((h + 3) / 4, n), dim3(256), 0, b->stream, b->d_desc, w, h, stride, p->delta_x, move_dp);
    }
    if (s.dp.form < 0) {
        HIPCK(hipGetLastError());
        return 0;
    }
    if (!fuse_e && !s.energy_beside) {
        ProfScope ps("emap_update", b->stream, 0);
        if ((rc = frozen_within_lag())) return rc;
        const int epoch = c0->frozen_epoch;
        const bool value = pb.value;
        const int nrg = plane_nrg(value, nrg_index(p->nrg_func)), nt = s.eu_nt;
#define CASE_NT(NT, N, V) if (nrg == N && value == V && nt == NT) hipLaunchKernelGGL((k_emap_update<N, NT, V>), dim3((h + EU_ROWS - 1) / EU_ROWS, n), dim3(64), 0, b->stream, b->d_desc, k, wnew, h, stride, log_index, epoch); else
#define CASE(N, V) K_EMAP_UPDATE_NT_FORMS(CASE_NT, N, V)
        K_EMAP_FORMS(CASE) return no_form("k_emap_update");
#undef CASE
#undef CASE_NT
    }
    if (s.full || s.band < 0) {
        ProfScope ps(s.full ? "dp_sweep" : "dp_update_tiled", b->stream, s.full ? 9.0 * wnew * h * n : 0);
        if ((rc = s.full ? launch_dp<false>(b, k, s.dp, rigm, wnew, h, leftright_next) : launch_dp<true>(b, k, s.dp, rigm, wnew, h, leftright_next))) return rc;
        HIPCK(hipGetLastError());
        return 0;
    }
    if (s.band == LQRHIP_CENSUS_BAND_LEVELS) {
        ProfScope ps("band_levels", b->stream, 0);
        if ((rc = launch_band_levels(b, k, wnew, h, leftright_next, s.levels_P, rigm))) return rc;
    } else if (s.band == LQRHIP_CENSUS_BAND_TW) {
        ProfScope ps("band_update", b->stream, 0);
        CENSUS(LQRHIP_CENSUS_BAND_TW);
#define CASE(LRV, RIGV) if ((leftright_next != 0) == LRV && (p->use_rigidity != 0) == RIGV) hipLaunchKernelGGL((k_band_update_tw<4, LRV, RIGV>), dim3(n), dim3(128 * 4), (size_t) 2 * h * sizeof(int), b->stream, b->d_desc, k, wnew, h, stride, g_dev_err); else
        K_LR_RIG_FORMS(CASE) return no_form("k_band_update_tw");
#undef CASE
    } else if (s.band == LQRHIP_CENSUS_BAND_MW8 || s.band == LQRHIP_CENSUS_BAND_MW16) {
        ProfScope ps("band_update", b->stream, 0);
        const int nw = s.band == LQRHIP_CENSUS_BAND_MW16 ? 16 : 8;
        CENSUS(nw == 16 ? LQRHIP_CENSUS_BAND_MW16 : LQRHIP_CENSUS_BAND_MW8);
#define CASE_NW(NWV, LRV, RIGV) if (nw == NWV && (leftright_next != 0) == LRV && (p->use_rigidity != 0) == RIGV) hipLaunchKernelGGL((k_band_update_mw<2, NWV, 8, LRV, RIGV>), dim3(n), dim3(64 * NWV), (size_t) h * sizeof(int), b->stream, b->d_desc, k, wnew, h, stride); else
#define CASE(LRV, RIGV) CASE_NW(8, LRV, RIGV) CASE_NW(16, LRV, RIGV)
        K_LR_RIG_FORMS(CASE) return no_form("k_band_update_mw");
#undef CASE
#undef CASE_NW
    } else {
        ProfScope ps("band_update", b->stream, 0);
        CENSUS(LQRHIP_CENSUS_BAND_GENERIC);
        hipLaunchKernelGGL(k_band_update, dim3(n), dim3(64), 0, b->stream, b->d_desc, k, wnew, h, stride, leftright_next);
    }
    {
        ProfScope ps("dp_update", b->stream, 0);
        if ((rc = launch_dp<true>(b, k, s.dp, rigm, wnew, h, leftright_next))) return rc;
    }
    HIPCK(hipGetLastError());
    return 0;
}

extern "C" int lqrhip_seam_log_reserve(LqrHipBatch *b, int n_seams, int h)
{
    int rc;
    if ((rc = pay_catchup(b))) return rc;
    for (auto *c : b->cs) if ((rc = ensure_log(c, n_seams, h))) return rc;
    return 0;
}

extern "C" int lqrhip_vs_commit(LqrHipBatch *b, int w0, int h0, int wc0, int n_seams, int first_level, int finish)
{
    int rc;
    if ((rc = batch_upload(b))) return rc;
    size_t lds = ((size_t) n_seams + wc0) * sizeof(int);
    if (lds > 150 * 1024) { g_err = "vs_commit: session too large for LDS"; return LQRHIP_EARG; }
    if (lds_needs_attr(lds)) {
// ... 226 lines not shown
{
#define LAUNCH_RV(DEEP) hipLaunchKernelGGL(k_compact<DEEP>, dim3(h0), dim3(256), 0, g_stream0, c->rgb0.get(), vs_of(c), (const float *) nullptr, (const float *) nullptr, \
                                           d, (float *) nullptr, (float *) nullptr, (int32_t *) nullptr, w0, w, (int) px_bytes(c), level, 0)
    if (px_bytes(c) > 4) LAUNCH_RV(true); else LAUNCH_RV(false);
#undef LAUNCH_RV
}
extern "C" int lqrhip_read_visible(LqrHipCarver *c, int w0, int h0, int w, int level, unsigned char *out)
{
    int rc = batch_sync_of(c);
    if (rc) return rc;
    size_t n = (size_t) w * h0 * px_bytes(c);
    Scratch tmp(g_stream0);
    uint8_t *d = tmp.get<uint8_t>(n, "&d", rc);
    if (rc) return rc;
    launch_read_visible(c, w0, h0, w, level, d);
    HIPCK(hipGetLastError());
    if ((rc = d2h_staged(out, d, n))) return rc;
    tmp.done();
    return 0;
}

extern "C" int lqrhip_read_visible_device(LqrHipCarver *c, int w0, int h0, int w, int level, void *device_out)
{
    int rc = batch_sync_of(c);
    if (rc) return rc;
    launch_read_visible(c, w0, h0, w, level, (uint8_t *) device_out);
    HIPCK(hipGetLastError());
    HIPCK(hipStreamSynchronize(g_stream0));
    return 0;
}

extern "C" int lqrhip_mask_line_max(const unsigned char *mask, int channels, int width, int height, int a0, int b0, int n_lines,
                                    int line_len, int direction)
{
    if (lqrhip_init() < 0) return LQRHIP_EHIP;
    if (n_lines <= 0 || line_len <= 0) return 0;
    int rc, result = 0;
    size_t bytes = (size_t) width * height * channels;
    Scratch tmp(g_stream0);
    uint8_t *d = tmp.get<uint8_t>(bytes, "&d", rc);
    if (rc) return rc;
    int *dout = tmp.get<int>(1, "&dout", rc);
    if (rc) return rc;
    HIPCK(hipMemcpyAsync(d, mask, bytes, hipMemcpyHostToDevice, g_stream0));
    HIPCK(hipMemsetAsync(dout, 0, sizeof(int), g_stream0));
    hipLaunchKernelGGL(k_mask_line_max, dim3(n_lines), dim3(256), 0, g_stream0, d, channels, width, a0, b0, line_len, direction, dout);
    HIPCK(hipGetLastError());
    HIPCK(hipMemcpyAsync(&result, dout, sizeof(int), hipMemcpyDeviceToHost, g_stream0));
    HIPCK(hipStreamSynchronize(g_stream0));
    tmp.done();
    return result;
}

extern "C" void lqrhip_pool_trim(void)
{
    (void) hipDeviceSynchronize();
    g_cache.trim();
    unpark_all();
}

extern "C" int lqrhip_device_sync(void)
{
    HIPCK(hipDeviceSynchronize());
    return check_dev_error();
}

extern "C" int lqrhip_read_vmap(LqrHipCarver *c, int w0, int h0, int w, int level, int depth, int *out)
{
    int rc = batch_sync_of(c);
    if (rc) return rc;
    size_t n = (size_t) w * h0;
    Scratch tmp(g_stream0);
    int32_t *d = tmp.get<int32_t>(n, "&d", rc);
    if (rc) return rc;
    hipLaunchKernelGGL(k_compact<false>, dim3(h0), dim3(256), 0, g_stream0, (const uint8_t *) nullptr, vs_of(c), (const float *) nullptr,
                       (const float *) nullptr, (uint8_t *) nullptr, (float *) nullptr, (float *) nullptr, d, w0, w, c->ch, level,
                       depth);
    HIPCK(hipGetLastError());
    if ((rc = d2h_staged(out, d, n * sizeof(int32_t)))) return rc;
    tmp.done();
    return 0;
}

extern "C" int lqrhip_read_working(LqrHipCarver *c, int w, int h, float *en, float *m, int *least_dx)
{
    int rc = batch_sync_of(c);
    if (rc) return rc;
    if (!c->wk.pix) return LQRHIP_EARG;
    int32_t fl[FLAG_COUNT];
    HIPCK(hipMemcpy(fl, c->wk.flags, sizeof fl, hipMemcpyDeviceToHost));
    const int org = fl[FLAG_ORG];
    size_t n = (size_t) c->stride * h;
    std::vector<float> t(n);
    std::vector<int8_t> tl(n);
    if (en) {
        HIPCK(hipMemcpy(t.data(), c->wk.en, n * sizeof(float), hipMemcpyDeviceToHost));
        for (int y = 0; y < h; y++) memcpy(en + (size_t) y * w, t.data() + (size_t) y * c->stride + org, (size_t) w * sizeof(float));
    }
    if (m) {
        HIPCK(hipMemcpy(t.data(), c->wk.m, n * sizeof(float), hipMemcpyDeviceToHost));
        for (int y = 0; y < h; y++) memcpy(m + (size_t) y * w, t.data() + (size_t) y * c->stride + org, (size_t) w * sizeof(float));
    }
    if (least_dx) {
        HIPCK(hipMemcpy(tl.data(), c->wk.least, n, hipMemcpyDeviceToHost));
        for (int y = 0; y < h; y++)
            for (int x = 0; x < w; x++) least_dx[(size_t) y * w + x] = y == 0 ? 0 : (int) tl[(size_t) y * c->stride + org + x];
    }
    return 0;
}

__global__ __launch_bounds__(256) void k_copy16(const u32x4 *__restrict__ src, u32x4 *__restrict__ dst, size_t n16);
static int reset_planes(LqrHipCarver *c, int w, int h)
{
    int rc = batch_sync_of(c);
    if (rc) return rc;
    const size_t n = (size_t) w * h;
    c->rgb0.reset(); c->vs.reset(); c->bias0.reset(); c->rig0.reset();
    if (c->wk.bias || c->wk.rig) { free_working(c); c->stride = 0; c->wk_h = 0; }
    c->w0 = w; c->h0 = h;
    drop_catchup(c);
    if ((rc = c->rgb0.alloc(n * px_bytes(c), "&c->rgb0")) || (rc = c->vs.alloc(n, "&c->vs"))) return rc;
    return 0;
}
extern "C" int lqrhip_carver_reset(LqrHipCarver *c, const void *device_rgb, int w, int h)
{
    if (!c || c->root || !c->aux.empty() || w < 1 || h < 1) return LQRHIP_EARG;
    int rc = reset_planes(c, w, h);
    if (rc) return rc;
    const size_t n = (size_t) w * h;
    {
        const size_t bytes = n * px_bytes(c), n16 = bytes / 16;
        if (n16 && !(((uintptr_t) device_rgb | (uintptr_t) c->rgb0.get()) & 15)) {
            hipLaunchKernelGGL(k_copy16, dim3((unsigned) ((n16 + 255) / 256)), dim3(256), 0, g_stream0, (const u32x4 *) device_rgb, (u32x4 *) c->rgb0.get(), n16);
            HIPCK(hipGetLastError());
            if (bytes & 15) HIPCK(hipMemcpyAsync(c->rgb0 + n16 * 16, (const uint8_t *) device_rgb + n16 * 16, bytes & 15, hipMemcpyDeviceToDevice, g_stream0));
        } else {
            HIPCK(hipMemcpyAsync(c->rgb0, device_rgb, bytes, hipMemcpyDeviceToDevice, g_stream0));
        }
    }
    HIPCK(hipMemsetAsync(c->vs, 0, n * sizeof(int32_t), g_stream0));
    if (c->batch) c->batch->dirty = true;
    if (c->active && (rc = ensure_working(c, w, h))) return rc;
    return 0;
}

enum { RESET_JOBS = 16 };
struct ResetJob { const uint8_t *src; uint8_t *dst; uint8_t *vs; size_t bytes; };
struct ResetJobs { ResetJob j[RESET_JOBS]; };
__global__ __launch_bounds__(256) void k_reset_jobs(const ResetJobs jobs, const size_t vs_bytes);
static int g_reset_batch_count = 0;
extern "C" int lqrhip_carver_reset_batch_count(void) { return g_reset_batch_count; }
extern "C" int lqrhip_carver_reset_batch(LqrHipCarver **cs, const void *const *device_rgb, int n, int w, int h)
{
    g_reset_batch_count = 0;
    if (!cs || !device_rgb || n < 1 || w < 1 || h < 1) return LQRHIP_EARG;
    for (int i = 0; i < n; i++)
        if (!cs[i] || cs[i]->root || !cs[i]->aux.empty() || !device_rgb[i]) return LQRHIP_EARG;
    const size_t npx = (size_t) w * h, vs_bytes = npx * sizeof(int32_t);
    ResetJobs jobs = {};
    int nj = 0;
    size_t most = vs_bytes;
    auto flush = [&]() -> int {
        if (!nj) return 0;
        const unsigned blocks = (unsigned) std::min<size_t>((most / 16 + 255) / 256 + 1, 4096);
        hipLaunchKernelGGL(k_reset_jobs, dim3(blocks, (unsigned) nj), dim3(256), 0, g_stream0, jobs, vs_bytes);
        nj = 0; most = vs_bytes;
// ... 136 lines not shown
```

gimp-lqr-plugin_amd/host/lqr_carver.c:

```c
#ifdef LQRHIP_TIMING
#define _POSIX_C_SOURCE 199309L
#endif
#include <stdlib.h>
#include <string.h>
#include <stdio.h>
#include <math.h>

#include "../../include/lqr.h"
#include "../../include/lqr_coldepth.h"
#include "../../include/lqr_imagetype.h"
#include "../../include/lqr_masks.h"
#include "../../include/lqr_energy.h"
#include "../../include/lqr_vmap.h"
#include "../../include/lqr_hip.h"
#include "lqr_mask_queue.h"
#include "lqr_sched.h"

#define MAXI(a, b) ((a) > (b) ? (a) : (b))
#define MINI(a, b) ((a) < (b) ? (a) : (b))

#ifdef LQRHIP_TIMING
#include <time.h>
enum { T_RELOAD, T_OPEN, T_CLOSE, T_TAIL, T_PARTS };
static double g_t_sum[T_PARTS];
static long g_t_calls[T_PARTS];
static double t_now(void) { struct timespec ts; clock_gettime(CLOCK_MONOTONIC, &ts); return ts.tv_sec * 1e3 + ts.tv_nsec * 1e-6; }
__attribute__((destructor)) static void t_report(void)
{
    static const char *const name[T_PARTS] = {"reload", "group_open", "group_close", "session_tail"};
    int i;
    for (i = 0; i < T_PARTS; i++)
        if (g_t_calls[i]) fprintf(stderr, "LQRHIP_TIMING %s calls %ld total_ms %.3f mean_ms %.4f\n", name[i], g_t_calls[i], g_t_sum[i], g_t_sum[i] / g_t_calls[i]);
}
#define T_BEGIN(part) const double t_begin_##part = t_now()
#define T_END(part) do { g_t_sum[part] += t_now() - t_begin_##part; g_t_calls[part]++; } while (0)
#else
#define T_BEGIN(part) do { } while (0)
#define T_END(part) do { } while (0)
#endif

struct _LqrProgress {
    gfloat update_step;
    LqrProgressFuncInit init;
    LqrProgressFuncUpdate update;
    LqrProgressFuncEnd end;
    gchar init_width_message[LQR_PROGRESS_MAX_MESSAGE_LENGTH];
    gchar end_width_message[LQR_PROGRESS_MAX_MESSAGE_LENGTH];
    gchar init_height_message[LQR_PROGRESS_MAX_MESSAGE_LENGTH];
    gchar end_height_message[LQR_PROGRESS_MAX_MESSAGE_LENGTH];
};

struct _LqrVMap {
    gint *buffer;
    gint width, height, depth, orientation;
};
struct _LqrVMapList {
    LqrVMap *current;
    LqrVMapList *next;
};
struct _LqrCarverList {
    LqrCarver *current;
    LqrCarverList *next;
};

struct _LqrCarver {
    LqrGeom geo;
    int channels;
    int col_depth;
    int image_type;
    int alpha_channel, black_channel;
    int preserve_input;
    int img_w, img_h;
    int active;
    LqrCarver *root;
    LqrCarverList *attached;

    int delta_x;
    float rigidity;
    float rigidity_map[2 * LQRHIP_MAX_DELTA + 1];
    int has_bias, has_rigmask;
    LqrMaskQueue mq[2];
    int nrg_func, nrg_radius;
    int leftright, lr_switch_frequency;
    float enl_step;
    int resize_order;
    int dump_vmaps;
    LqrVMapList *flushed_vs;
    LqrProgress *progress;
    int session_update_step, session_rescale_total, session_rescale_current;

    LqrHipCarver *dev;
    LqrHipBatch *own_batch;
    int wk_valid;

    guchar *ro_image;
    size_t ro_image_len;
    guchar *in_buffer;
    size_t in_buffer_len;
    int ro_valid, ro_line, ro_x;
    guchar *ro_buffer;
    int ro_buffer_len;

    float *dbg_en, *dbg_m;
    int *dbg_least, dbg_w, dbg_h;
};

static const int k_depth_bytes[4] = {1, 2, 4, 8};
#define PX_BYTES(r) ((size_t) (r)->channels * k_depth_bytes[(r)->col_depth])

#define MAX_SUB 8
typedef struct {
    LqrCarver **r;
    int n;
    LqrHipBatch *b[MAX_SUB];
    int nb;
} Group;

static int g_debug_snapshot = 0;
void lqrx_set_debug(gint on) { g_debug_snapshot = on; }

static int g_last_rc = 0;
static LqrRetVal hip_ret(int rc)
{
    if (rc == 0) return LQR_OK;
    g_last_rc = rc;
    fprintf(stderr, "liblqr-hip: device error %d: %s\n", rc, lqrhip_last_error());
    return rc == LQRHIP_ENOMEM ? LQR_NOMEM : LQR_ERROR;
}
#define HIP_CATCH(expr) LQR_CATCH(hip_ret(expr))

LqrProgress *lqr_progress_new(void)
{
    LqrProgress *p = (LqrProgress *) calloc(1, sizeof *p);
    if (!p) return NULL;
    p->update_step = 0.02f;
    strcpy(p->init_width_message, "Resizing width...");
    strcpy(p->init_height_message, "Resizing height...");
    strcpy(p->end_width_message, "done");
    strcpy(p->end_height_message, "done");
    return p;
}
LqrRetVal lqr_progress_set_init(LqrProgress *p, LqrProgressFuncInit f) { p->init = f; return LQR_OK; }
LqrRetVal lqr_progress_set_update(LqrProgress *p, LqrProgressFuncUpdate f) { p->update = f; return LQR_OK; }
LqrRetVal lqr_progress_set_end(LqrProgress *p, LqrProgressFuncEnd f) { p->end = f; return LQR_OK; }
LqrRetVal lqr_progress_set_update_step(LqrProgress *p, gfloat s) { p->update_step = s; return LQR_OK; }
static LqrRetVal copy_message(gchar *dst, const gchar *src)
{
    if (!src) return LQR_ERROR;
    snprintf(dst, LQR_PROGRESS_MAX_MESSAGE_LENGTH, "%s", src);
    return LQR_OK;
}
LqrRetVal lqr_progress_set_init_width_message(LqrProgress *p, const gchar *m) { return copy_message(p->init_width_message, m); }
LqrRetVal lqr_progress_set_init_height_message(LqrProgress *p, const gchar *m) { return copy_message(p->init_height_message, m); }
LqrRetVal lqr_progress_set_end_width_message(LqrProgress *p, const gchar *m) { return copy_message(p->end_width_message, m); }
LqrRetVal lqr_progress_set_end_height_message(LqrProgress *p, const gchar *m) { return copy_message(p->end_height_message, m); }

#define LIST_APPEND(T, head, n)                      \
    do {                                             \
        T **pp__ = &(head);                          \
        while (*pp__) pp__ = &(*pp__)->next;         \
        *pp__ = (n);                                 \
    } while (0)
LqrCarverList *lqr_carver_list_start(LqrCarver *r) { return r->attached; }
LqrCarver *lqr_carver_list_current(LqrCarverList *l) { return l->current; }
LqrCarverList *lqr_carver_list_next(LqrCarverList *l) { return l->next; }
LqrVMapList *lqr_vmap_list_start(LqrCarver *r) { return r->flushed_vs; }
LqrVMap *lqr_vmap_list_current(LqrVMapList *l) { return l->current; }
LqrVMapList *lqr_vmap_list_next(LqrVMapList *l) { return l->next; }
LqrRetVal lqr_vmap_list_foreach(LqrVMapList *list, LqrVMapFunc func, gpointer data)
{
    for (; list; list = list->next) LQR_CATCH(func(list->current, data));
    return LQR_OK;
}
gint *lqr_vmap_get_data(LqrVMap *v) { return v->buffer; }
gint lqr_vmap_get_width(LqrVMap *v) { return v->width; }
gint lqr_vmap_get_height(LqrVMap *v) { return v->height; }
gint lqr_vmap_get_depth(LqrVMap *v) { return v->depth; }
gint lqr_vmap_get_orientation(LqrVMap *v) { return v->orientation; }
void lqr_vmap_destroy(LqrVMap *v) { if (v) { free(v->buffer); free(v); } }
LqrVMap *lqr_vmap_new(gint *buffer, gint width, gint height, gint depth, gint orientation)
{
    LqrVMap *v = (LqrVMap *) calloc(1, sizeof *v);
    if (!v) return NULL;
    v->buffer = buffer;
    v->width = width; v->height = height; v->depth = depth; v->orientation = orientation;
    return v;
}
// ... 424 lines not shown
}
LqrRetVal lqr_carver_rigmask_add_area(LqrCarver *r, gdouble *buffer, gint width, gint height, gint x_off, gint y_off)
{
    return mask_add_f(r, buffer, LQR_COLDEPTH_64F, 0, 1, 0, width, height, x_off, y_off);
}
LqrRetVal lqr_carver_rigmask_add(LqrCarver *r, gdouble *buffer)
{
    return lqr_carver_rigmask_add_area(r, buffer, lqr_carver_get_width(r), lqr_carver_get_height(r), 0, 0);
}
LqrRetVal lqr_carver_rigmask_add_rgb(LqrCarver *r, guchar *rgb, gint channels)
{
    return lqr_carver_rigmask_add_rgb_area(r, rgb, channels, lqr_carver_get_width(r), lqr_carver_get_height(r), 0, 0);
}
LqrRetVal lqrx_carver_bias_add_area_device(LqrCarver *r, const void *device_buffer, LqrColDepth depth, gint bias_factor, gint width, gint height,
                                           gint x_off, gint y_off)
{
    if (depth != LQR_COLDEPTH_32F && depth != LQR_COLDEPTH_64F) return LQR_ERROR;
    return mask_add_f(r, device_buffer, (int) depth, 1, 0, bias_factor, width, height, x_off, y_off);
}
LqrRetVal lqrx_carver_rigmask_add_area_device(LqrCarver *r, const void *device_buffer, LqrColDepth depth, gint width, gint height, gint x_off,
                                              gint y_off)
{
    if (depth != LQR_COLDEPTH_32F && depth != LQR_COLDEPTH_64F) return LQR_ERROR;
    return mask_add_f(r, device_buffer, (int) depth, 1, 1, 0, width, height, x_off, y_off);
}

static LqrRetVal mask_add_xy(LqrCarver *r, int is_rig, double v, int x, int y)
{
    LqrMaskQueue *q = &r->mq[is_rig];
    int rc, index;
    if (!q->n) {
        LQR_CATCH(is_rig ? mask_prepare(r) : bias_prepare(r));
        if (x < 0 || y < 0 || x >= lqr_carver_get_width(r) || y >= lqr_carver_get_height(r)) return LQR_ERROR;
        HIP_CATCH(lqrhip_mask_plane_ensure(r->dev, is_rig));
        if (is_rig) r->has_rigmask = 1; else r->has_bias = 1;
        r->wk_valid = 0;
    } else if (x < 0 || y < 0 || x >= lqr_carver_get_width(r) || y >= lqr_carver_get_height(r))
        return LQR_ERROR;
    index = r->geo.transposed ? x * r->geo.w0 + y : y * r->geo.w0 + x;
    rc = lqr_maskq_append(q, (size_t) r->geo.w0 * r->geo.h0, index, v);
    if (rc == LQR_MASKQ_FULL) {
        LQR_CATCH(mask_queue_flush_one(r, is_rig));
        rc = lqr_maskq_append(q, (size_t) r->geo.w0 * r->geo.h0, index, v);
    }
    return rc == LQR_MASKQ_OK ? LQR_OK : rc == LQR_MASKQ_NOMEM ? LQR_NOMEM : LQR_ERROR;
}
LqrRetVal lqr_carver_bias_add_xy(LqrCarver *r, gdouble bias, gint x, gint y)
{
    if (bias == 0) return LQR_OK;
    return mask_add_xy(r, 0, bias, x, y);
}
LqrRetVal lqr_carver_rigmask_add_xy(LqrCarver *r, gdouble rigidity, gint x, gint y) { return mask_add_xy(r, 1, rigidity, x, y); }

static void mask_clear(LqrCarver *r, int is_rig)
{
    lqr_maskq_reset(&r->mq[is_rig]);
    (void) hip_ret(lqrhip_mask_clear(r->dev, is_rig));
    if (is_rig) r->has_rigmask = 0; else r->has_bias = 0;
    r->wk_valid = 0;
}
void lqr_carver_bias_clear(LqrCarver *r) { mask_clear(r, 0); }
void lqr_carver_rigmask_clear(LqrCarver *r) { mask_clear(r, 1); }

static LqrRetVal mask_read(LqrCarver *r, int is_rig, gfloat *out)
{
    LQR_CATCH(mask_queue_flush(r));
    if (lqr_geom_needs_flatten(&r->geo)) return LQR_ERROR;
    HIP_CATCH(lqrhip_read_mask_plane(r->dev, is_rig, r->geo.transposed, out));
    return LQR_OK;
}
LqrRetVal lqrx_carver_get_bias(LqrCarver *r, gfloat *out) { return mask_read(r, 0, out); }
LqrRetVal lqrx_carver_get_rigmask(LqrCarver *r, gfloat *out) { return mask_read(r, 1, out); }

static LqrRetVal take_debug_snapshot(LqrCarver *r)
{
    size_t n = (size_t) r->geo.w * r->geo.h;
    free(r->dbg_en); free(r->dbg_m); free(r->dbg_least);
    r->dbg_w = r->geo.w; r->dbg_h = r->geo.h;
    r->dbg_en = (float *) malloc(n * sizeof(float));
    r->dbg_m = (float *) malloc(n * sizeof(float));
    r->dbg_least = (int *) malloc(n * sizeof(int));
    if (!r->dbg_en || !r->dbg_m || !r->dbg_least) return LQR_NOMEM;
    HIP_CATCH(lqrhip_read_working(r->dev, r->geo.w, r->geo.h, r->dbg_en, r->dbg_m, r->dbg_least));
    return LQR_OK;
}

static LqrRetVal group_build_vsmap(Group *g, const LqrSession *s, int *reported)
{
    LqrCarver *r0 = g->r[0];
    LqrHipDpParams p;
    int l, i;
    dp_params(r0, &p);
    HIP_ALL(g, lqrhip_seam_log_reserve(B, s->n_seams, r0->geo.h));

    for (l = s->max_level; l < s->depth; l++) {
        const int lr_pick = r0->leftright;
        LqrSeam seam;
        lqr_session_seam(s, l, &seam);
        if (seam.report && r0->progress && r0->progress->update) {
            HIP_ALL(g, lqrhip_batch_sync(B));
            if (l > *reported) {
                r0->progress->update(seam.fraction);
                *reported = l;
            }
        }
        if (seam.full)
            for (i = 0; i < g->n; i++) g->r[i]->leftright ^= 1;
        HIP_ALL(g, lqrhip_seam_step(B, &p, seam.w_before, r0->geo.h, l - s->max_level, lr_pick, seam.full, r0->leftright));
        for (i = 0; i < g->n; i++) { g->r[i]->geo.level++; g->r[i]->geo.w--; }
    }

    if (g_debug_snapshot)
        for (i = 0; i < g->n; i++) LQR_CATCH(take_debug_snapshot(g->r[i]));

    T_BEGIN(T_TAIL);
    HIP_ALL(g, lqrhip_session_check(B, r0->geo.h, s->wc0, s->n_seams, r0->delta_x));
    HIP_ALL(g, lqrhip_batch_sync(B));
    HIP_ALL(g, lqrhip_vs_commit(B, r0->geo.w0, r0->geo.h0, s->wc0, s->n_seams, s->first_level, s->finish));
    HIP_ALL(g, lqrhip_inflate(B, r0->geo.w0, r0->geo.h0, s->depth - 1, s->max_level));
    HIP_ALL(g, lqrhip_planes_commit(B));
    T_END(T_TAIL);
    FOR_TREE(g, i, r, {
        lqr_geom_session_done(&r->geo, s->depth, s->n_seams);
        ro_invalidate(r);
    });
    return LQR_OK;
}

static LqrRetVal session_run(Group *g, const LqrSession *s, int redo, int *reported)
{
    LqrCarver *r0 = g->r[0];
    LqrHipDpParams p;
    int i;
    for (i = 0; i < g->n; i++) set_width_one(g->r[i], s->wc0);
    dp_params(r0, &p);
    if (!r0->wk_valid || redo) {
        const int from_visible = (r0->geo.max_level != 1 || r0->geo.w0 != r0->geo.w_start);
        if (from_visible) HIP_ALL(g, lqrhip_wk_init(B, 1));
        else HIP_ALL(g, lqrhip_wk_init_emap(B, &p, r0->geo.w, r0->geo.h));
        for (i = 0; i < g->n; i++) g->r[i]->wk_valid = 1;
        if (from_visible) HIP_ALL(g, lqrhip_emap_build(B, &p, r0->geo.w, r0->geo.h));
    } else
        HIP_ALL(g, lqrhip_emap_build(B, &p, r0->geo.w, r0->geo.h));
    HIP_ALL(g, lqrhip_mmap_build(B, &p, r0->geo.w, r0->geo.h, r0->leftright));
    return group_build_vsmap(g, s, reported);
}

static LqrRetVal group_build_maps(Group *g, int depth)
{
    LqrCarver *r0 = g->r[0];
    LqrSession s;
    LqrRetVal ret;
    int i, k, reported = -1, *snap;
    if (depth <= r0->geo.max_level) return LQR_OK;
    if (!r0->active || r0->root) return LQR_ERROR;
    lqr_session_begin(&s, r0->geo.max_level, depth, r0->geo.w_start - r0->geo.max_level + 1, r0->lr_switch_frequency, r0->session_rescale_current,
                      r0->session_rescale_total, r0->session_update_step);
    snap = (int *) malloc((size_t) g->n * 3 * sizeof *snap);
    if (!snap) return LQR_NOMEM;
    for (i = 0; i < g->n; i++) { snap[3 * i] = g->r[i]->geo.w; snap[3 * i + 1] = g->r[i]->geo.level; snap[3 * i + 2] = g->r[i]->leftright; }
    g_last_rc = 0;
    ret = session_run(g, &s, 0, &reported);
    for (k = 0; k < 2 && ret != LQR_OK; k++) {
        const int fault = (ret == LQR_ERROR && g_last_rc == LQRHIP_EFAULT);
        if (fault || g_last_rc == LQRHIP_ENOMEM)
            for (i = 0; i < g->nb; i++) (void) lqrhip_session_rollback(g->b[i], r0->geo.w0, r0->geo.h0, s.first_level, s.finish);
// ... 376 lines not shown
        r->flushed_vs = NULL;
        lqr_geom_reset(&r->geo, r->img_w, r->img_h);
        r->leftright = 0;
        r->has_bias = r->has_rigmask = 0;
        r->wk_valid = 0;
        ro_invalidate(r);
        if (r->active) rigidity_table(r);
    }
    HIP_CATCH(rc);
    HIP_CATCH(lqrhip_reset_sync());
    T_END(T_RELOAD);
    return LQR_OK;
}

gint lqrx_guess_new_size(const guchar *mask, gint channels, gint width, gint height, gint x_off, gint y_off,
                         gint old_width, gint old_height, gint direction)
{
    int lw = MINI(old_width, width + x_off) - MAXI(0, x_off);
    int lh = MINI(old_height, height + y_off) - MAXI(0, y_off);
    int old_size = direction ? old_height : old_width, m;
    if (direction == 0)
        m = lqrhip_mask_line_max(mask, channels, width, height, MAXI(0, y_off) - y_off, MAXI(0, -x_off),
                                 MINI(old_height, height + y_off) - MAXI(0, y_off), lw, 0);
    else
        m = lqrhip_mask_line_max(mask, channels, width, height, MAXI(0, x_off) - x_off, MAXI(0, -y_off),
                                 MINI(old_width, width + x_off) - MAXI(0, x_off), lh, 1);
    if (m < 0) { fprintf(stderr, "liblqr-hip: guess_new_size failed: %s\n", lqrhip_last_error()); return old_size; }
    return old_size - m;
}

static LqrRetVal energy_run(LqrCarver *r, void *buffer, int on_device, int orientation, int form, int depth, int image_type)
{
    Group g;
    LqrHipDpParams p;
    LqrRetVal ret = LQR_OK;
    if (r->root) return LQR_ERROR;
    LQR_CATCH(mask_queue_flush(r));
    LQR_CATCH(group_open(&g, &r, 1));
    if (r->geo.w != r->geo.w_start - r->geo.max_level + 1) ret = group_flatten(&g);
    if (ret == LQR_OK && form >= 0 && r->geo.transposed != orientation) ret = group_transpose(&g);
    if (ret == LQR_OK && !r->wk_valid) {
        if ((ret = hip_ret(lqrhip_wk_init(g.b[0], r->geo.max_level != 1 || r->geo.w0 != r->geo.w_start))) == LQR_OK) r->wk_valid = 1;
    }
    if (ret == LQR_OK) {
        dp_params(r, &p);
        ret = hip_ret(lqrhip_emap_build(g.b[0], &p, r->geo.w, r->geo.h));
    }
    if (ret == LQR_OK)
        ret = hip_ret(form < 0 ? lqrhip_read_working(r->dev, r->geo.w, r->geo.h, (float *) buffer, NULL, NULL)
                               : lqrhip_energy_out(g.b[0], r->geo.w, r->geo.h, r->geo.transposed, form, depth, image_type, buffer, on_device));
    group_close(&g);
    return ret;
}
LqrRetVal lqrx_carver_get_energy(LqrCarver *r, gfloat *buffer) { return energy_run(r, buffer, 0, 0, -1, 0, 0); }

static LqrRetVal energy_read(LqrCarver *r, void *buffer, int on_device, int orientation, int form, int depth, int image_type)
{
    if (!r || !buffer || (orientation != 0 && orientation != 1)) return LQR_ERROR;
    if (form == 2 && (depth < LQR_COLDEPTH_8I || depth > LQR_COLDEPTH_64F || image_type < LQR_RGB_IMAGE || image_type >= LQR_CUSTOM_IMAGE))
        return LQR_ERROR;
    return energy_run(r, buffer, on_device, orientation, form, depth, image_type);
}
LqrRetVal lqr_carver_get_energy(LqrCarver *r, gfloat *buffer, gint orientation) { return energy_read(r, buffer, 0, orientation, 1, 0, 0); }
LqrRetVal lqr_carver_get_true_energy(LqrCarver *r, gfloat *buffer, gint orientation) { return energy_read(r, buffer, 0, orientation, 0, 0, 0); }
LqrRetVal lqr_carver_get_energy_image(LqrCarver *r, void *buffer, gint orientation, LqrColDepth col_depth, LqrImageType image_type)
{
    return energy_read(r, buffer, 0, orientation, 2, (int) col_depth, (int) image_type);
}
LqrRetVal lqrx_carver_get_energy_device(LqrCarver *r, void *device_buffer, gint orientation, gint normalised)
{
    return energy_read(r, device_buffer, 1, orientation, normalised ? 1 : 0, 0, 0);
}
LqrRetVal lqrx_carver_get_energy_image_device(LqrCarver *r, void *device_buffer, gint orientation, LqrColDepth col_depth, LqrImageType image_type)
{
    return energy_read(r, device_buffer, 1, orientation, 2, (int) col_depth, (int) image_type);
}

LqrRetVal lqrx_carver_debug_maps(LqrCarver *r, gfloat *en, gfloat *m, gint *least_dx)
{
    if (!r->active || !r->wk_valid) return LQR_ERROR;
    HIP_CATCH(lqrhip_read_working(r->dev, r->geo.w, r->geo.h, en, m, least_dx));
    return LQR_OK;
}
gint lqrx_carver_debug_width(LqrCarver *r) { return r->dbg_w; }
gint lqrx_carver_debug_height(LqrCarver *r) { return r->dbg_h; }
LqrRetVal lqrx_carver_debug_snapshot(LqrCarver *r, gfloat *en, gfloat *m, gint *least_dx)
{
    size_t n = (size_t) r->dbg_w * r->dbg_h;
    if (!r->dbg_m) return LQR_ERROR;
    if (en) memcpy(en, r->dbg_en, n * sizeof(float));
    if (m) memcpy(m, r->dbg_m, n * sizeof(float));
    if (least_dx) memcpy(least_dx, r->dbg_least, n * sizeof(int));
    return LQR_OK;
}
```

include/lqr_hip.h:

```cpp
#ifndef LQR_HIP_H
#define LQR_HIP_H

#include <stddef.h>

#ifdef __cplusplus
extern "C" {
#endif

#define LQRHIP_OK 0
#define LQRHIP_ENOMEM (-2)
#define LQRHIP_EHIP (-1)
#define LQRHIP_EARG (-3)
#define LQRHIP_EFAULT (-4)
#define LQRHIP_EMAP (-5)
#define LQRHIP_MAX_DELTA 16
#define LQRHIP_MAX_CHANNELS 64
#define LQRHIP_MAX_FRAME_WIDTH 16384

typedef struct LqrHipCarver LqrHipCarver;
typedef struct LqrHipBatch LqrHipBatch;

typedef struct LqrHipDpParams {
    int delta_x;
    int use_rigidity;
// ... 4 lines not shown
} LqrHipDpParams;

int lqrhip_init(void);
const char *lqrhip_last_error(void);

LqrHipCarver *lqrhip_carver_create(const unsigned char *rgb, int w, int h, int channels);
LqrHipCarver *lqrhip_carver_create_ext(const void *rgb, int w, int h, int channels, int depth);
int lqrhip_carver_set_read_luma(LqrHipCarver *c, int luma);
int lqrhip_carver_set_read(LqrHipCarver *c, int image_type, int alpha, int black);
void lqrhip_carver_destroy(LqrHipCarver *c);
int lqrhip_carver_reset(LqrHipCarver *c, const void *device_rgb, int w, int h);
int lqrhip_carver_reset_batch(LqrHipCarver **cs, const void *const *device_rgb, int n, int w, int h);
int lqrhip_carver_reset_batch_count(void);
int lqrhip_reset_sync(void);
int lqrhip_carver_attach(LqrHipCarver *root, LqrHipCarver *aux);
int lqrhip_carver_activate(LqrHipCarver *c);

int lqrhip_mask_add(LqrHipCarver *c, const unsigned char *mask, int channels, int width, int height,
                    int x_off, int y_off, int transposed, int is_rigmask, int bias_factor);

int lqrhip_mask_add_f(LqrHipCarver *c, const void *mask, int depth, int on_device, int width, int height, int x_off, int y_off,
                      int transposed, int is_rigmask, int bias_factor);
int lqrhip_mask_plane_ensure(LqrHipCarver *c, int is_rigmask);
int lqrhip_mask_scatter(LqrHipCarver *c, int is_rigmask, const int *index, const double *value, const size_t *start, int buckets);
int lqrhip_mask_clear(LqrHipCarver *c, int is_rigmask);
int lqrhip_read_mask_plane(LqrHipCarver *c, int is_rigmask, int transposed, float *out);
unsigned long long lqrhip_debug_mask_flushes(void);

int lqrhip_sub_batches(int n);
int lqrhip_general_batch_limit(int w);
int lqrhip_general_batch_limit_delta(int w, int delta_x);
void lqrhip_set_sub_batches(int n);
LqrHipBatch *lqrhip_batch_create(LqrHipCarver **carvers, int n);
void lqrhip_batch_set_shared(LqrHipBatch *b, int shared);
void lqrhip_batch_destroy(LqrHipBatch *b);
int lqrhip_batch_sync(LqrHipBatch *b);
void lqrhip_batch_abort(LqrHipBatch *b);
void *lqrhip_batch_stream(LqrHipBatch *b);

int lqrhip_wk_init(LqrHipBatch *b, int from_visible);
int lqrhip_emap_build(LqrHipBatch *b, const LqrHipDpParams *p, int w, int h);
int lqrhip_wk_init_emap(LqrHipBatch *b, const LqrHipDpParams *p, int w, int h);
int lqrhip_energy_out(LqrHipBatch *b, int w, int h, int transposed, int form, int depth, int image_type, void *out, int on_device);
int lqrhip_mmap_build(LqrHipBatch *b, const LqrHipDpParams *p, int w, int h, int leftright);
int lqrhip_seam_step(LqrHipBatch *b, const LqrHipDpParams *p, int w, int h, int log_index,
                     int leftright_pick, int full_rebuild, int leftright_next);
int lqrhip_seam_log_reserve(LqrHipBatch *b, int n_seams, int h);
int lqrhip_vs_commit(LqrHipBatch *b, int w0, int h0, int wc0, int n_seams, int first_level, int finish);
int lqrhip_session_check(LqrHipBatch *b, int h, int wc0, int n_seams, int delta_x);
void lqrhip_set_selfcheck(int on);
void lqrhip_set_recovery(int on);
int lqrhip_get_recovery(void);
int lqrhip_session_rollback(LqrHipBatch *b, int w0, int h0, int first_level, int finish);
void lqrhip_batch_set_safe(LqrHipBatch *b, int safe);
void lqrhip_set_no_spin(int on);
int lqrhip_get_no_spin(void);
int lqrhip_fault_stats(unsigned long long *out8, int reset);
void lqrhip_debug_inject(int kind, int at_step, int times);
void lqrhip_debug_fail_alloc(int nth);
unsigned long long lqrhip_debug_pool_live(void);
void lqrhip_debug_fixedcost(unsigned long long out4[4], int reset);
int lqrhip_inflate(LqrHipBatch *b, int w0, int h0, int l, int max_level);
typedef struct LqrHipVMap LqrHipVMap;
int lqrhip_vmap_stage(const int *map, int on_device, int width, int height, int depth, int orientation, LqrHipVMap **out);
int lqrhip_vmap_load(LqrHipBatch *b, const LqrHipVMap *m);
void lqrhip_vmap_release(LqrHipVMap *m);
int lqrhip_flatten(LqrHipBatch *b, int w0, int h0, int w, int level);
int lqrhip_transpose(LqrHipBatch *b, int w, int h);
int lqrhip_planes_commit(LqrHipBatch *b);
int lqrhip_inflate_commit(LqrHipBatch *b);

int lqrhip_read_visible(LqrHipCarver *c, int w0, int h0, int w, int level, unsigned char *out);
int lqrhip_mask_line_max(const unsigned char *mask, int channels, int width, int height, int a0, int b0, int n_lines, int line_len,
                         int direction);
int lqrhip_read_visible_device(LqrHipCarver *c, int w0, int h0, int w, int level, void *device_out);
int lqrhip_device_sync(void);
int lqrhip_mem_info(unsigned long long *free_bytes, unsigned long long *total_bytes, unsigned long long *cached_bytes);
int lqrhip_copy_bandwidth(unsigned long long bytes, int iters, double *gbps);
int lqrhip_vmap_to_rgba(const int *vmap, int w, int h, int depth, const double col_start[3], const double col_end[3],
                        unsigned char *out_rgba);
void lqrhip_pool_trim(void);
int lqrhip_read_vmap(LqrHipCarver *c, int w0, int h0, int w, int level, int depth, int *out);
int lqrhip_read_working(LqrHipCarver *c, int w, int h, float *en, float *m, int *least_dx);

void lqrhip_prof_enable(int on);
void lqrhip_set_update_mode(int mode);
void lqrhip_set_sweep_threads(int n);
void lqrhip_set_carve_fused(int max_images);
void lqrhip_set_carve_beside(int mode);
unsigned long long lqrhip_carve_beside_launches(int reset);
void lqrhip_set_vpath_mode(int mode, int par_max);
void lqrhip_set_dp_persistent_limit(int workgroups);
void lqrhip_set_dp_persistent_px(int px);
void lqrhip_prof_reset(void);
int lqrhip_prof_get(const char *kernel, double *ms_total, long long *launches, double *bytes_total);
int lqrhip_prof_get_union(const char *kernel, double *ms_union);
int lqrhip_moved_bytes(unsigned long long *bytes, int reset);
void lqrhip_set_band_levels(int slots);
int lqrhip_band_levels_stats(unsigned long long *out8, int reset);
enum {
    LQRHIP_CENSUS_VP_PARALLEL = 0,
    LQRHIP_CENSUS_VPATH1 = 1,
    LQRHIP_CENSUS_VPATH = 2,
    LQRHIP_CENSUS_CARVE_E = 3,
    LQRHIP_CENSUS_CARVE = 4,
    LQRHIP_CENSUS_TILE_P_G3 = 5,
    LQRHIP_CENSUS_TILE_P_G2 = 6,
    LQRHIP_CENSUS_TILE_P_G4 = 7,
    LQRHIP_CENSUS_TILE_P_GENERAL = 8,
    LQRHIP_CENSUS_DP_TILE = 9,
    LQRHIP_CENSUS_BAND_LEVELS = 10,
    LQRHIP_CENSUS_BAND_TW = 11,
    LQRHIP_CENSUS_BAND_MW8 = 12,
    LQRHIP_CENSUS_BAND_MW16 = 13,
    LQRHIP_CENSUS_BAND_GENERIC = 14,
    LQRHIP_CENSUS_SWEEP = 15,
    LQRHIP_CENSUS_SWEEP_FULL = 25,
    LQRHIP_CENSUS_SWEEP_UPDATE = 26,
    LQRHIP_CENSUS_LDS_ATTR_SWEEP = 27,
    LQRHIP_CENSUS_LDS_ATTR_COMMIT = 28,
    LQRHIP_CENSUS_SLOTS = 32
};
int lqrhip_launch_census(unsigned long long *out, int n, int reset);

#ifdef __cplusplus
}
#endif
#endif
```

Before: 540,600 Mseams*px/s.

## Fuse seam backtrack with carve and energy update via on-device work list

```diff
diff --git a/gimp-lqr-plugin_amd/csrc/k_backtrack.hip b/gimp-lqr-plugin_amd/csrc/k_backtrack.hip
--- a/gimp-lqr-plugin_amd/csrc/k_backtrack.hip
+++ b/gimp-lqr-plugin_amd/csrc/k_backtrack.hip
@@ -1,50 +1,7 @@
 #include "lqr_common.h"
 #include "lqr_kernels.h"
-
-__device__ __forceinline__ int row_argmin(const gf32 *mrow, int w, int lr, float *s_val, int *s_idx)
-{
-    const int tid = threadIdx.x;
-    const float INF = __int_as_float(0x7f800000);
-    float bv = INF;
-    int bi = -1;
-    for (int base = 0; base < w; base += 16 * VPATH_THREADS) {
-        f32x4 v[4];
-#pragma unroll
-        for (int i = 0; i < 4; i++) {
-            const int x = base + 4 * (tid + VPATH_THREADS * i);
-            if (x + 3 < w) v[i] = *(const GLOBAL_AS f32x4 *) (mrow + x);
-            else { v[i] = (f32x4) {INF, INF, INF, INF}; for (int j = 0; j < 4; j++) if (x + j < w) v[i][j] = mrow[x + j]; }
-        }
-#pragma unroll
-        for (int i = 0; i < 4; i++)
-#pragma unroll
-            for (int j = 0; j < 4; j++) {
-                const int x = base + 4 * (tid + VPATH_THREADS * i) + j;
-                const float f = v[i][j];
-                if (x < w && (f < bv || (f == bv && lr))) { bv = f; bi = x; }
-            }
-    }
-    auto better = [&](float v2, int i2, float v1, int i1) {
-        if (i2 < 0) return false;
-        if (i1 < 0) return true;
-        if (v2 < v1) return true;
-        if (v2 > v1) return false;
-        return lr ? (i2 > i1) : (i2 < i1);
-    };
-    for (int o = 32; o > 0; o >>= 1) {
-        const float v2 = __shfl_xor(bv, o);
-        const int i2 = __shfl_xor(bi, o);
-        if (better(v2, i2, bv, bi)) { bv = v2; bi = i2; }
-    }
-    if ((tid & 63) == 0) { s_val[tid >> 6] = bv; s_idx[tid >> 6] = bi; }
-    __syncthreads();
-    bv = s_val[0]; bi = s_idx[0];
-#pragma unroll
-    for (int k = 1; k < VPATH_THREADS / 64; k++) if (better(s_val[k], s_idx[k], bv, bi)) { bv = s_val[k]; bi = s_idx[k]; }
-    const float lim = 536870912.0f;
-    const bool ok = (bi >= 0) && (bv < lim || (bv == lim && lr));
-    return ok ? bi : -1;
-}
+#include "lqr_walk.h"
+
 
 __device__ unsigned long long g_moved_bytes;
 __device__ __forceinline__ void publish_side(const GCarver &c, int org, int acc, int w, int h, int lane, int moved_unit)
@@ -64,6 +21,11 @@
     if (hipMemcpyFromSymbol(out, HIP_SYMBOL(g_moved_bytes), sizeof(unsigned long long)) != hipSuccess) return -1;
     if (reset) { unsigned long long z = 0; (void) hipMemcpyToSymbol(HIP_SYMBOL(g_moved_bytes), &z, sizeof z); }
     return 0;
+}
+unsigned long long *lqr_moved_bytes_dev(void)
+{
+    void *p = nullptr;
+    return hipGetSymbolAddress(&p, HIP_SYMBOL(g_moved_bytes)) == hipSuccess ? (unsigned long long *) p : nullptr;
 }
 
 __global__ __launch_bounds__(VPATH_THREADS) void k_vpath(const DevCarver *cs, int w, int h, int stride, int lr, int delta,
@@ -127,20 +89,6 @@
     publish_side(c, org, acc, w, h, lane, moved_unit);
 }
 
-constexpr int vp1_rows(int delta) { return delta == 1 ? 28 : delta == 2 ? 12 : delta == 3 ? 8 : 4; }
-#define VP1_AHEAD 3
-template <int r>
-__device__ __forceinline__ void vp1_step(const int e, int &o, int &path)
-{
-    asm volatile("v_writelane_b32 %0, %1, %2" : "+v"(path) : "s"(o), "n"(r));
-    o += __builtin_amdgcn_readlane(e, o);
-}
-template <int N, int... Rs>
-__device__ __forceinline__ void vp1_chase(const int (&e)[N], int &o, int &path, std::integer_sequence<int, Rs...>)
-{
-    (vp1_step<Rs>(e[Rs], o, path), ...);
-}
-
 template <int DELTA>
 __global__ __launch_bounds__(VPATH_THREADS) void k_vpath1(const DevCarver *cs, int w, int h, int stride, int lr, int log_index, int moved_unit)
 {
@@ -159,57 +107,12 @@
     const int lane = tid;
     gi32 *seam = c.seam_x;
     gi32 *logp = c.seam_log + (size_t) log_index * h;
-    constexpr int R = VP1_ROWS, NB = VP1_AHEAD + 1, RL = VP1_ROWS / 4;
-    static_assert(VP1_ROWS % 4 == 0 && VP1_ROWS * DELTA <= 28 && VP1_AHEAD * VP1_ROWS * DELTA + 32 <= 120, "window margin");
-    u32x4 regs[NB][RL];
-    int xa[NB];
-    auto window_base = [&](int cx) { return (cx - 120) & ~15; };
-    auto load_chunk = [&](int b, int y_top, int cx) {
-        const int base = window_base(cx);
-        xa[b] = base;
-        const int voff = min(max(base + 16 * (lane & 15), 0), stride - 16);
-        const int rsub = (lane >> 4) * stride;
-#pragma unroll
-        for (int q = 0; q < RL; q++) {
-            const int row = max((y_top - 4 * q) * stride - rsub, stride);
-            regs[b][q] = *(const GLOBAL_AS u32x4 *) (c.least + (unsigned) (row + voff));
-        }
-    };
     int acc = 0;
-    auto run_chunk = [&](int b, int y_top) {
-        const int relbase = x - 32 - xa[b];
-        int e[R];
-#pragma unroll
-        for (int q = 0; q < RL; q++) *(u32x4 *) (s_win + q * 1024 + lane * 16) = regs[b][q];
-        __builtin_amdgcn_wave_barrier();
-#pragma unroll
-        for (int r = 0; r < R; r++) e[r] = s_win[r * 256 + relbase + lane];
-        int e2[R / 2];
-#pragma unroll
-        for (int k = 0; k < R / 2; k++) e2[k] = e[2 * k] + __builtin_amdgcn_ds_bpermute((lane + e[2 * k]) << 2, e[2 * k + 1]);
-        int o = 32, path = 0;
-        vp1_chase<R / 2>(e2, o, path, std::make_integer_sequence<int, R / 2>{});
-        const int odd = path + s_win[min(lane, R / 2 - 1) * 512 + relbase + path];
-        __builtin_amdgcn_wave_barrier();
-        const int pe = path + x - 32, po = odd + x - 32;
-        const int nrows = min(R, y_top);
-        if (2 * lane < nrows) { seam[y_top - 2 * lane] = pe; logp[y_top - 2 * lane] = pe; acc += pe; }
+#define VP1_RECORD(y_top, nrows, pe, po) \
+        if (2 * lane < nrows) { seam[y_top - 2 * lane] = pe; logp[y_top - 2 * lane] = pe; acc += pe; } \
         if (2 * lane + 1 < nrows) { seam[y_top - 2 * lane - 1] = po; logp[y_top - 2 * lane - 1] = po; acc += po; }
-        x = (nrows == R) ? x + o - 32 : __builtin_amdgcn_readlane((nrows & 1) ? po : pe, nrows >> 1);
-    };
-    int y_top = h - 1;
-#pragma unroll
-    for (int k = 0; k < VP1_AHEAD; k++) load_chunk(k, y_top - k * R, x);
-    while (true) {
-#pragma unroll
-        for (int k = 0; k < NB; k++) {
-            load_chunk((k + VP1_AHEAD) % NB, y_top - VP1_AHEAD * R, x);
-            run_chunk(k, y_top);
-            y_top -= R;
-            if (y_top < 1) break;
-        }
-        if (y_top < 1) break;
-    }
+#include "vpath1_walk.inc"
+#undef VP1_RECORD
     if (lane == 0) { seam[0] = x; logp[0] = x; acc += x; }
     publish_side(c, org, acc, w, h, lane, moved_unit);
 }
diff --git a/gimp-lqr-plugin_amd/csrc/k_carve.hip b/gimp-lqr-plugin_amd/csrc/k_carve.hip
--- a/gimp-lqr-plugin_amd/csrc/k_carve.hip
+++ b/gimp-lqr-plugin_amd/csrc/k_carve.hip
@@ -1,5 +1,6 @@
 #include "lqr_common.h"
 #include "lqr_kernels.h"
+#include "lqr_walk.h"
 
 
 #ifndef CG
@@ -193,19 +194,19 @@
     }
 }
 
-template <bool BESIDE>
-__device__ __forceinline__ void carve_row(const GCarver &c, int org, int side, int y, int w, int stride, int delta, int move_dp, int lane, int h = 0, int radius = 0)
+template <bool BESIDE, class SR = SeamPlain>
+__device__ __forceinline__ void carve_row(const GCarver &c, int org, int side, int y, int w, int stride, int delta, int move_dp, int lane, int h = 0, int radius = 0, SR sr = SR())
 {
     const int wnew = w - 1;
     int pa = 0x7fffffff, pb = -1;
     if (BESIDE) {
         int xmin, xmax;
-        nrg_interval(c.seam_x, y, h, wnew, radius, xmin, xmax);
+        nrg_interval(c.seam_x, y, h, wnew, radius, xmin, xmax, sr);
         if (xmin <= xmax) { pa = org + side + xmin; pb = org + side + xmax; }
     }
-    const int v = c.seam_x[y];
+    const int v = sr(c.seam_x + y);
     const size_t ro = (size_t) y * stride;
-    const int vprev = y > 0 ? c.seam_x[y - 1] : 0;
+    const int vprev = y > 0 ? sr(c.seam_x + (y - 1)) : 0;
     gu32 *en = (gu32 *) (c.en + ro), *mm = (gu32 *) (c.m + ro), *l32 = (gu32 *) (c.least + ro);
     gu32 *rg = c.rig ? (gu32 *) (c.rig + ro) : (gu32 *) nullptr;
     if (side == 0) {
@@ -339,8 +340,143 @@
     if (y < h) carve_row<true>(c, org, side, y, w, stride, p.delta, move_dp, threadIdx.x & 63, h, p.radius);
 }
 
+static_assert(BB_EU_ROWS == EU_ROWS, "lqr_beside.h restates EU_ROWS");
+typedef GLOBAL_AS unsigned long long gu64;
+#ifdef LQR_TIMING
+__device__ unsigned long long g_walk_cycles[2];
+extern "C" int lqrhip_walk_timing(unsigned long long *out) { (void) hipDeviceSynchronize(); return hipMemcpyFromSymbol(out, HIP_SYMBOL(g_walk_cycles), sizeof(unsigned long long) * 2) == hipSuccess ? 0 : -1; }
+#endif
+__device__ __forceinline__ void st_wt(gi32 *p, int v) { __hip_atomic_store(p, v, __ATOMIC_RELAXED, __HIP_MEMORY_SCOPE_AGENT); }
+
+template <int NRG, int DELTA>
+__global__ __launch_bounds__(256) __attribute__((amdgpu_waves_per_eu(5))) void k_carve_v(const DevCarver *cs, DpK p, int w, int h, int stride, int lr, int move_dp, int k, int epoch, int n,
+                                                 int moved_unit, unsigned tag, unsigned long long *list, unsigned long long *moved_bytes, int *dev_err)
+{
+    const int eblk = bb_energy_entries(h), rblk = bb_carve_entries(h);
+    const unsigned total = (unsigned) n * (unsigned) (eblk + rblk);
+    gu64 *entries = (gu64 *) list + BB_LIST_HEAD;
+    const int tid = threadIdx.x;
+    if ((int) blockIdx.x < n) {
+        __shared__ float s_val[VPATH_THREADS / 64];
+        __shared__ int s_idx[VPATH_THREADS / 64];
+        __shared__ int s_path[BB_MAX_ROWS];
+        __shared__ int s_lo;
+        __shared__ __attribute__((aligned(16))) int8_t s_win[BB_WALK_ROWS * 256];
+        const int img = blockIdx.x;
+        const GCarver c = gview(cs[img]);
+        const int org = c.flags[FLAG_ORG];
+        if (tid == 0) {
+            s_lo = h;
+            if (img == 0) __hip_atomic_store((gu64 *) list + ((tag + 1) & 1), 0ull, __ATOMIC_RELAXED, __HIP_MEMORY_SCOPE_AGENT);
+        }
+        const int xmin = row_argmin(c.m + (size_t) (h - 1) * stride, w, lr, s_val, s_idx);
+        if (tid >= 128) return;
+        const int lane = tid & 63;
+#ifdef LQR_TIMING
+        const unsigned long long t0 = __builtin_amdgcn_s_memrealtime();
+#endif
+        if (tid < 64) {
+            int x = __builtin_amdgcn_readfirstlane(max(xmin, 0));
+            __builtin_amdgcn_s_setprio(3);
+            constexpr int VP1_ROWS = BB_WALK_ROWS;
+#define VP1_RECORD(y_top, nrows, pe, po) \
+            if (2 * lane < nrows) LDS_FLAG(s_path[y_top - 2 * lane]) = pe; \
+            if (2 * lane + 1 < nrows) LDS_FLAG(s_path[y_top - 2 * lane - 1]) = po; \
+            LDS_FLAG(s_lo) = y_top - nrows + 1;
+#include "vpath1_walk.inc"
+#undef VP1_RECORD
+            LDS_FLAG(s_path[0]) = x;
+            LDS_FLAG(s_lo) = 0;
+#ifdef LQR_TIMING
+            if (img == 0 && lane == 0) g_walk_cycles[0] = __builtin_amdgcn_s_memrealtime() - t0;
+#endif
+            return;
+        }
+        gi32 *seam = c.seam_x, *logp = c.seam_log + (size_t) k * h;
+        gu64 *tail = (gu64 *) list + (tag & 1);
+        int done = h, acc = 0, side = -1, next_q = rblk - 1, next_e = eblk - 1;
+        for (unsigned spins = 0; done > 0;) {
+            const int lo = __builtin_amdgcn_readfirstlane(LDS_FLAG(s_lo));
+            if (lo >= done) {
+                __builtin_amdgcn_s_sleep(2);
+                if (++spins > (1u << 24)) { if (lane == 0) dev_fail(dev_err, DEVERR_TILE_TIMEOUT); return; }
+                continue;
+            }
+            for (int y = done - 1 - lane; y >= lo; y -= 64) { const int v = LDS_FLAG(s_path[y]); st_wt(seam + y, v); st_wt(logp + y, v); acc += v; }
+            const int xlo = __builtin_amdgcn_readfirstlane(LDS_FLAG(s_path[lo]));
+            asm volatile("s_waitcnt vmcnt(0)" ::: "memory");
+            done = lo;
+            if (side < 0) {
+                int S = acc;
+                for (int o = 32; o > 0; o >>= 1) S += __shfl_xor(S, o);
+                side = bb_side_bound(S, xlo, lo, DELTA, w, h);
+                if (side >= 0 && lane == 0) { c.flags[FLAG_ORG_PREV] = org; c.flags[FLAG_SIDE] = side; c.flags[FLAG_ORG] = org + side; c.flags[FLAG_OVF_ROW] = h; }
+            }
+            if (side < 0) continue;
+            const int e0 = bb_first_eblk(lo, p.radius), q0 = bb_first_quad(lo, p.radius);
+            const int ne = max(next_e - e0 + 1, 0), nq = max(next_q - q0 + 1, 0), cnt = ne + nq;
+            if (cnt == 0) continue;
+            unsigned base = 0;
+            if (lane == 0) base = (unsigned) __hip_atomic_fetch_add(tail, (unsigned long long) cnt, __ATOMIC_RELAXED, __HIP_MEMORY_SCOPE_AGENT);
+            base = (unsigned) __builtin_amdgcn_readfirstlane((int) base);
+            for (int i = lane; i < cnt; i += 64) {
+                const bool en = i < ne;
+                const unsigned slot = base + (unsigned) i;
+                if (slot < total)
+                    __hip_atomic_store(entries + slot, bb_pack(tag, en ? 1 : 0, img, en ? next_e - i : next_q - (i - ne), side, org), __ATOMIC_RELAXED, __HIP_MEMORY_SCOPE_AGENT);
+            }
+            next_e -= ne; next_q -= nq;
+        }
+        for (int o = 32; o > 0; o >>= 1) acc += __shfl_xor(acc, o);
+        if (lane == 0) {
+            const long long all = (long long) h * (w - 1);
+            atomicAdd(moved_bytes, (unsigned long long) (side ? (long long) acc : all - acc) * (unsigned long long) moved_unit);
+#ifdef LQR_TIMING
+            if (img == 0) g_walk_cycles[1] = __builtin_amdgcn_s_memrealtime() - t0;
+#endif
+        }
+        return;
+    }
+    __shared__ unsigned long long s_entry;
+    if (tid == 0) {
+        gu64 *src = entries + (blockIdx.x - (unsigned) n);
+        unsigned long long e = 0;
+        for (unsigned sp = 0;;) {
+            e = __hip_atomic_load(src, __ATOMIC_RELAXED, __HIP_MEMORY_SCOPE_AGENT);
+            if ((unsigned) (e >> BB_TAG_SHIFT) == tag) break;
+            e = 0;
+            if (sp < 16) __builtin_amdgcn_s_sleep(4); else __builtin_amdgcn_s_sleep(32);
+            ++sp;
+            if ((sp & 255) == 0 && dev_failed(dev_err)) break;
+            if (sp > (1u << 18)) { dev_fail(dev_err, DEVERR_TILE_TIMEOUT); break; }
+        }
+        s_entry = e;
+    }
+    __syncthreads();
+    const unsigned long long ew = ((unsigned long long) (unsigned) __builtin_amdgcn_readfirstlane((int) (s_entry >> 32)) << 32) | (unsigned) __builtin_amdgcn_readfirstlane((int) s_entry);
+    if (ew == 0) return;
+    const BbEntry e = bb_unpack(ew);
+    if (e.image >= n) return;
+    if (e.energy) {
+        PixRead<false> rd;
+        rd.setup(tid, 256);
+        if (tid >= 64 || e.index >= eblk) return;
+        GCarver c = gview_phys(cs[e.image]);
+        c.en += e.org + e.side;
+        emap_update_block<NRG, 12, false, true>(c, rd, p, w - 1, h, stride, k, epoch, (unsigned) e.index, tid, SeamLive());
+        return;
+    }
+    GCarver c = gview_phys(cs[e.image]);
+    c.en = uni_ptr(c.en); c.m = uni_ptr(c.m); c.least = uni_ptr(c.least); c.seam_x = uni_ptr(c.seam_x);
+    const int y = e.index * 4 + (tid >> 6);
+    if (y < h) carve_row<true>(c, e.org, e.side, y, w, stride, DELTA, move_dp, tid & 63, h, p.radius, SeamLive());
+}
+
 #define INST(N) template __global__ void k_carve_u<N>(const DevCarver *, DpK, int, int, int, int, int, int, int);
 K_CARVE_U_FORMS(INST)
+#undef INST
+#define INST(N, D) template __global__ void k_carve_v<N, D>(const DevCarver *, DpK, int, int, int, int, int, int, int, int, int, unsigned, unsigned long long *, unsigned long long *, int *);
+K_CARVE_V_FORMS(INST)
 #undef INST
 #define INST(N) template __global__ void k_carve_e<N>(const DevCarver *, DpK, int, int, int, int, int, int);
 K_CARVE_E_FORMS(INST)
diff --git a/gimp-lqr-plugin_amd/csrc/lqr_beside.h b/gimp-lqr-plugin_amd/csrc/lqr_beside.h
--- /dev/null
+++ b/gimp-lqr-plugin_amd/csrc/lqr_beside.h
@@ -0,0 +1,48 @@
+#pragma once
+#include <stdint.h>
+
+constexpr int BB_WALK_ROWS = 12;
+constexpr int BB_MAX_ROWS = 4096;
+constexpr int BB_MAX_IMAGES = 1024;
+constexpr int BB_EU_ROWS = 62;
+constexpr int BB_MIN_ROWS = 3 * BB_WALK_ROWS + 1;
+
+constexpr long long bb_min_ll(long long a, long long b) { return a < b ? a : b; }
+constexpr long long bb_rem_min(long long x, long long r, long long delta)
+{
+    const long long k0 = delta > 0 ? bb_min_ll(r, x / delta) : r;
+    return k0 * x - delta * (k0 * (k0 + 1) / 2);
+}
+constexpr long long bb_rem_max(long long x, long long r, long long delta, long long w)
+{
+    const long long k1 = delta > 0 ? bb_min_ll(r, (w - 1 - x) / delta) : r;
+    return k1 * x + delta * (k1 * (k1 + 1) / 2) + (r - k1) * (w - 1);
+}
+constexpr int bb_side_bound(long long S, int x, int r, int delta, int w, int h)
+{
+    const long long all = (long long) h * (w - 1);
+    if (2 * (S + bb_rem_max(x, r, delta, w)) < all) return 1;
+    if (2 * (S + bb_rem_min(x, r, delta)) >= all) return 0;
+    return -1;
+}
+
+constexpr int BB_TAG_SHIFT = 38;
+constexpr unsigned BB_EPOCHS = (1u << 26) - 2;
+constexpr unsigned bb_tag(unsigned launches) { return 1u + launches % BB_EPOCHS; }
+struct BbEntry { unsigned tag; int energy, image, index, side, org; };
+constexpr uint64_t bb_pack(unsigned tag, int energy, int image, int index, int side, int org)
+{
+    return ((uint64_t) tag << BB_TAG_SHIFT) | ((uint64_t) (energy & 1) << 37) | ((uint64_t) (image & 1023) << 27) |
+           ((uint64_t) (index & 4095) << 15) | ((uint64_t) (side & 1) << 14) | (uint64_t) (org & 16383);
+}
+constexpr BbEntry bb_unpack(uint64_t e)
+{
+    return BbEntry{(unsigned) (e >> BB_TAG_SHIFT), (int) ((e >> 37) & 1), (int) ((e >> 27) & 1023), (int) ((e >> 15) & 4095), (int) ((e >> 14) & 1), (int) (e & 16383)};
+}
+
+constexpr int BB_LIST_HEAD = 2;
+constexpr int bb_carve_entries(int h) { return (h + 3) / 4; }
+constexpr int bb_energy_entries(int h) { return (h + BB_EU_ROWS - 1) / BB_EU_ROWS; }
+constexpr long long bb_entries(int n, int h) { return (long long) n * (bb_carve_entries(h) + bb_energy_entries(h)); }
+constexpr int bb_first_quad(int lo, int radius) { return lo <= 0 ? 0 : (lo + 1 + radius + 3) / 4; }
+constexpr int bb_first_eblk(int lo, int radius) { return lo <= 0 ? 0 : (lo + 2 + radius + BB_EU_ROWS - 1) / BB_EU_ROWS; }
diff --git a/gimp-lqr-plugin_amd/csrc/lqr_common.h b/gimp-lqr-plugin_amd/csrc/lqr_common.h
--- a/gimp-lqr-plugin_amd/csrc/lqr_common.h
+++ b/gimp-lqr-plugin_amd/csrc/lqr_common.h
@@ -210,17 +210,32 @@
     return r + off;
 }
 
-__device__ __forceinline__ void nrg_interval(const gi32 *seam, int y, int h, int w, int radius, int &xmin, int &xmax)
+struct SeamPlain {
+    static constexpr bool live = false;
+    __device__ __forceinline__ int operator()(const gi32 *p) const { return *p; }
+};
+struct SeamLive {
+    static constexpr bool live = true;
+    __device__ __forceinline__ int operator()(const gi32 *p) const { return __hip_atomic_load(p, __ATOMIC_RELAXED, __HIP_MEMORY_SCOPE_AGENT); }
+};
+
+template <class SR>
+__device__ __forceinline__ void nrg_interval(const gi32 *seam, int y, int h, int w, int radius, int &xmin, int &xmax, SR sr)
 {
     int y1a = max(y - radius, 0), y1b = min(y + radius, h - 1);
-    int lo = seam[y], hi = seam[y] - 1;
+    const int v = sr(seam + y);
+    int lo = v, hi = v - 1;
     for (int y1 = y1a; y1 <= y1b; y1++) {
-        int x = seam[y1];
+        int x = sr(seam + y1);
         lo = min(lo, x - radius);
         hi = max(hi, x + radius - 1);
     }
     xmin = max(0, lo);
     xmax = min(w - 1, hi);
+}
+__device__ __forceinline__ void nrg_interval(const gi32 *seam, int y, int h, int w, int radius, int &xmin, int &xmax)
+{
+    nrg_interval(seam, y, h, w, radius, xmin, xmax, SeamPlain());
 }
 
 template <bool LR, bool RIG, bool UPDATE, bool MASK>
diff --git a/gimp-lqr-plugin_amd/csrc/lqr_kernels.h b/gimp-lqr-plugin_amd/csrc/lqr_kernels.h
--- a/gimp-lqr-plugin_amd/csrc/lqr_kernels.h
+++ b/gimp-lqr-plugin_amd/csrc/lqr_kernels.h
@@ -19,6 +19,7 @@
 #define K_VPATH1_FORMS(X) X(1) X(2) X(3) X(4) X(5) X(6) X(7)
 #define K_VP_FORMS(X) K_VPATH1_FORMS(X) X(8) X(9) X(10)
 template <int DELTA> __global__ __launch_bounds__(VPATH_THREADS) void k_vpath1(const DevCarver *cs, int w, int h, int stride, int lr, int log_index, int moved_unit);
+unsigned long long *lqr_moved_bytes_dev(void);
 
 template <int DELTA> __global__ __launch_bounds__(256) void k_vp_maps(const DevCarver *cs, int w, int h, int stride);
 template <int DELTA> __global__ __launch_bounds__(VPATH_THREADS) void k_vp_solve(const DevCarver *cs, int w, int h, int stride, int lr, int log_index, int moved_unit);
@@ -28,6 +29,10 @@
 template <int NRG> __global__ __launch_bounds__(256) void k_carve_e(const DevCarver *cs, DpK p, int w, int h, int stride, int move_dp, int k, int epoch);
 #define K_CARVE_U_FORMS(X) X(0) X(1) X(2) X(3) X(4) X(5) X(6)
 template <int NRG> __global__ __launch_bounds__(256) void k_carve_u(const DevCarver *cs, DpK p, int w, int h, int stride, int move_dp, int k, int epoch, int n);
+#define K_CARVE_V_DELTAS(X) X(1) X(2)
+#define K_CARVE_V_FORMS(X) X(0, 1) X(1, 1) X(2, 1) X(3, 1) X(4, 1) X(5, 1) X(6, 1) X(0, 2) X(1, 2) X(2, 2) X(3, 2) X(4, 2) X(5, 2) X(6, 2)
+template <int NRG, int DELTA> __global__ __launch_bounds__(256) __attribute__((amdgpu_waves_per_eu(5))) void k_carve_v(const DevCarver *cs, DpK p, int w, int h, int stride, int lr, int move_dp, int k, int epoch, int n,
+                                                                                  int moved_unit, unsigned tag, unsigned long long *list, unsigned long long *moved_bytes, int *dev_err);
 
 #define K_DP_SWEEP_PXT_FORMS(X) X(1) X(2) X(4) X(8) X(16)
 #define K_LR_RIG_FORMS(X) X(false, false) X(false, true) X(true, false) X(true, true)
diff --git a/gimp-lqr-plugin_amd/csrc/lqr_pixel.h b/gimp-lqr-plugin_amd/csrc/lqr_pixel.h
--- a/gimp-lqr-plugin_amd/csrc/lqr_pixel.h
+++ b/gimp-lqr-plugin_amd/csrc/lqr_pixel.h
@@ -22,8 +22,8 @@
     __device__ __forceinline__ double operator()(const gu32 *pix, size_t o, int, bool) const { return ((const gf64 *) pix)[o]; }
 };
 
-template <int NRG, int EU_NT, bool VALUE, bool ONE_WAVE>
-__device__ __forceinline__ void emap_update_block(const GCarver c, const PixRead<VALUE> rd, const DpK p, int w, int h, int stride, int k, int epoch, unsigned blk, int tid)
+template <int NRG, int EU_NT, bool VALUE, bool ONE_WAVE, class SR = SeamPlain>
+__device__ __forceinline__ void emap_update_block(const GCarver c, const PixRead<VALUE> rd, const DpK p, int w, int h, int stride, int k, int epoch, unsigned blk, int tid, SR sr = SR())
 {
     __shared__ double bt[64][EU_NT];
     __shared__ float bb[64][EU_NT];
@@ -33,10 +33,10 @@
     constexpr bool luma = (NRG >= 3);
     int xmin = 0, xmax = -1, lo = 0;
     if (row_ok) {
-        nrg_interval(c.seam_x, y, h, w, p.radius, xmin, xmax);
+        nrg_interval(c.seam_x, y, h, w, p.radius, xmin, xmax, sr);
         int l = xmin - 1, r = xmax + 1;
-        if (y > 0) { int a, b; nrg_interval(c.seam_x, y - 1, h, w, p.radius, a, b); if (b >= a) { l = min(l, a); r = max(r, b); } }
-        if (y < h - 1) { int a, b; nrg_interval(c.seam_x, y + 1, h, w, p.radius, a, b); if (b >= a) { l = min(l, a); r = max(r, b); } }
+        if (y > 0) { int a, b; nrg_interval(c.seam_x, y - 1, h, w, p.radius, a, b, sr); if (b >= a) { l = min(l, a); r = max(r, b); } }
+        if (y < h - 1) { int a, b; nrg_interval(c.seam_x, y + 1, h, w, p.radius, a, b, sr); if (b >= a) { l = min(l, a); r = max(r, b); } }
         lo = max(l, 0);
         int pos[EU_NT];
 #pragma unroll
@@ -45,7 +45,10 @@
         for (int j = k; j >= epoch; j -= EU_LOGB) {
             int v[EU_LOGB];
 #pragma unroll
-            for (int u = 0; u < EU_LOGB; u++) v[u] = lg[(size_t) max(j - u, epoch) * h];
+            for (int u = 0; u < EU_LOGB; u++) {
+                const gi32 *q = lg + (size_t) max(j - u, epoch) * h;
+                if (SR::live && u == 0 && j == k) v[u] = sr(q); else v[u] = *q;
+            }
 #pragma unroll
             for (int u = 0; u < EU_LOGB; u++) {
                 const int vu = (j - u >= epoch) ? v[u] : 0x7fffffff;
diff --git a/gimp-lqr-plugin_amd/csrc/lqr_plan.h b/gimp-lqr-plugin_amd/csrc/lqr_plan.h
--- a/gimp-lqr-plugin_amd/csrc/lqr_plan.h
+++ b/gimp-lqr-plugin_amd/csrc/lqr_plan.h
@@ -2,6 +2,7 @@
 #include <algorithm>
 #include <stddef.h>
 #include "../../include/lqr_hip.h"
+#include "lqr_beside.h"
 
 #define DP_THREADS 1024
 constexpr int dppx_px(int px) { return px == 3 ? 2 : px; }
@@ -38,6 +39,7 @@
     int sweep_threads = 256;
     int carve_fused = 4;
     int carve_beside = -1;
+    int backtrack_beside = -1;
     int update_mode = -1;
     int band_levels = -1;
     int dpp_limit = -1;
@@ -71,6 +73,7 @@
     int vp_rows = 0, vp_chunks = 0;
     int carve = 0;
     bool energy_beside = false;
+    bool backtrack_beside = false;
     bool catchup = false;
     int eu_nt = 0;
     bool full = false;
@@ -155,6 +158,14 @@
 {
     if (k.carve_beside == 0 || delta > 2 || b.value || wnew <= 1) return false;
     return k.carve_beside > 0 || (!b.shared && b.group() >= (size_t) CARVE_BESIDE_MIN);
+}
+
+constexpr int BACKTRACK_BESIDE_MIN = 8;
+static inline bool plan_backtrack_beside(const PlanKnobs &k, const PlanBatch &b, int delta, int h, bool energy_beside, int backtrack, bool catchup)
+{
+    if (k.backtrack_beside == 0 || !energy_beside || backtrack != LQRHIP_CENSUS_VPATH1 || delta < 1 || delta > 2 || !b.spin || catchup) return false;
+    if (h < BB_MIN_ROWS || h > BB_MAX_ROWS || b.images > BB_MAX_IMAGES) return false;
+    return k.backtrack_beside > 0 || (!b.shared && b.group() >= (size_t) BACKTRACK_BESIDE_MIN);
 }
 
 static inline StepPlan plan_seam_step(const PlanKnobs &k, const PlanDevice &d, const PlanBatch &b, int delta, bool use_rig, int w, int h, bool full_rebuild, int lag)
@@ -170,6 +181,7 @@
     s.carve = delta <= 2 && b.group() <= (size_t) k.carve_fused && wnew > 1 && !b.value ? LQRHIP_CENSUS_CARVE_E : LQRHIP_CENSUS_CARVE;
     s.energy_beside = s.carve == LQRHIP_CENSUS_CARVE && plan_carve_beside(k, b, delta, wnew);
     s.catchup = lag > frozen_lag(b.images);
+    s.backtrack_beside = plan_backtrack_beside(k, b, delta, h, s.energy_beside, s.backtrack, s.catchup);
     s.eu_nt = eu_samples(delta);
     if (wnew <= 1) return s;
     if (full_rebuild) {
diff --git a/gimp-lqr-plugin_amd/csrc/lqr_shim.hip b/gimp-lqr-plugin_amd/csrc/lqr_shim.hip
--- a/gimp-lqr-plugin_amd/csrc/lqr_shim.hip
+++ b/gimp-lqr-plugin_amd/csrc/lqr_shim.hip
@@ -113,6 +113,8 @@
     DevBuf<unsigned long long> exch;
     int exch_ntiles = 0, exch_n = 0, exch_px = 0;
     int tile_epoch = 0;
+    DevBuf<unsigned long long> wlist;
+    unsigned wlist_launches = 0;
     bool dirty = true;
     int shared_n = 1;
     bool shared = false;
@@ -962,6 +964,14 @@
 {
     const unsigned long long v = g_carve_beside_launches;
     if (reset) g_carve_beside_launches = 0;
+    return v;
+}
+extern "C" void lqrhip_set_backtrack_beside(int mode) { g_knobs.backtrack_beside = mode < 0 ? -1 : mode ? 1 : 0; }
+static unsigned long long g_backtrack_beside_launches;
+extern "C" unsigned long long lqrhip_backtrack_beside_launches(int reset)
+{
+    const unsigned long long v = g_backtrack_beside_launches;
+    if (reset) g_backtrack_beside_launches = 0;
     return v;
 }
 extern "C" void lqrhip_set_update_mode(int mode) { g_knobs.update_mode = mode; }
@@ -1228,7 +1238,7 @@
                 hipLaunchKernelGGL(k_vp_maps<delta>, dim3((w + 255) / 256, nchunks, n), dim3(256), 0, b->stream, b->d_desc, w, h, stride);
                 hipLaunchKernelGGL(k_vp_solve<delta>, dim3(n), dim3(VPATH_THREADS), (size_t) (nchunks + 2) * sizeof(int), b->stream, b->d_desc, w, h, stride, leftright_pick, log_index, moved_unit);
             })) return no_form("k_vp_maps");
-    } else {
+    } else if (!s.backtrack_beside) {
         ProfScope ps("vpath", b->stream, 0);
         CENSUS(s.backtrack);
         if (!with_listed(K_VPATH1_FORMS, p->delta_x, [&](auto delta) {
@@ -1247,6 +1257,32 @@
         if (!with_listed(K_CARVE_E_FORMS, nrg_index(p->nrg_func), [&](auto nrg) {
                 hipLaunchKernelGGL((k_carve_e<nrg>), dim3((h + 3) / 4, n), dim3(256), 0, b->stream, b->d_desc, k, w, h, stride, move_dp, log_index, epoch);
             })) return no_form("k_carve_e");
+    } else if (s.backtrack_beside) {
+        const int epoch = c0->frozen_epoch;
+        const size_t need = (size_t) BB_LIST_HEAD + (size_t) bb_entries((int) n, h);
+        if (b->wlist.size() < need) {
+            bool grew = false;
+            HIPCK(hipStreamSynchronize(b->stream));
+            if ((rc = b->wlist.ensure(need, "&b->wlist", &grew))) return rc;
+            HIPCK(hipMemsetAsync(b->wlist, 0, need * sizeof(unsigned long long), b->stream));
+        }
+        unsigned long long *moved = lqr_moved_bytes_dev();
+        if (!moved) { g_err = "k_carve_v: no address for the moved-bytes counter"; return LQRHIP_EHIP; }
+        const unsigned tag = bb_tag(b->wlist_launches++);
+        ProfScope ps("carve", b->stream, 4.0 * (double) w * h * n);
+        CENSUS(LQRHIP_CENSUS_VPATH1);
+        CENSUS(LQRHIP_CENSUS_CARVE);
+        g_carve_beside_launches++;
+        g_backtrack_beside_launches++;
+        const unsigned grid = n + (unsigned) bb_entries((int) n, h);
+        bool launched = false;
+        with_listed(K_CARVE_U_FORMS, nrg_index(p->nrg_func), [&](auto nrg) {
+            launched = with_listed(K_CARVE_V_DELTAS, p->delta_x, [&](auto delta) {
+                hipLaunchKernelGGL((k_carve_v<nrg, delta>), dim3(grid), dim3(256), 0, b->stream, b->d_desc, k, w, h, stride, leftright_pick, move_dp, log_index, epoch,
+                                   (int) n, moved_unit, tag, b->wlist.get(), moved, g_dev_err);
+            });
+        });
+        if (!launched) return no_form("k_carve_v");
     } else if (s.energy_beside) {
         if ((rc = frozen_within_lag())) return rc;
         const int epoch = c0->frozen_epoch;
@@ -1639,6 +1675,16 @@
     return 0;
 }
 
+extern "C" int lqrhip_read_seam_flags(LqrHipCarver *c, int *org, int *org_prev, int *side)
+{
+    int rc = batch_sync_of(c);
+    if (rc) return rc;
+    if (!c->wk.flags) return LQRHIP_EARG;
+    int32_t fl[FLAG_COUNT];
+    HIPCK(hipMemcpy(fl, c->wk.flags, sizeof fl, hipMemcpyDeviceToHost));
+    *org = fl[FLAG_ORG]; *org_prev = fl[FLAG_ORG_PREV]; *side = fl[FLAG_SIDE];
+    return 0;
+}
 extern "C" int lqrhip_read_working(LqrHipCarver *c, int w, int h, float *en, float *m, int *least_dx)
 {
     int rc = batch_sync_of(c);
diff --git a/gimp-lqr-plugin_amd/csrc/lqr_walk.h b/gimp-lqr-plugin_amd/csrc/lqr_walk.h
--- /dev/null
+++ b/gimp-lqr-plugin_amd/csrc/lqr_walk.h
@@ -0,0 +1,61 @@
+#pragma once
+#include "lqr_common.h"
+
+__device__ __forceinline__ int row_argmin(const gf32 *mrow, int w, int lr, float *s_val, int *s_idx)
+{
+    const int tid = threadIdx.x;
+    const float INF = __int_as_float(0x7f800000);
+    float bv = INF;
+    int bi = -1;
+    for (int base = 0; base < w; base += 16 * VPATH_THREADS) {
+        f32x4 v[4];
+#pragma unroll
+        for (int i = 0; i < 4; i++) {
+            const int x = base + 4 * (tid + VPATH_THREADS * i);
+            if (x + 3 < w) v[i] = *(const GLOBAL_AS f32x4 *) (mrow + x);
+            else { v[i] = (f32x4) {INF, INF, INF, INF}; for (int j = 0; j < 4; j++) if (x + j < w) v[i][j] = mrow[x + j]; }
+        }
+#pragma unroll
+        for (int i = 0; i < 4; i++)
+#pragma unroll
+            for (int j = 0; j < 4; j++) {
+                const int x = base + 4 * (tid + VPATH_THREADS * i) + j;
+                const float f = v[i][j];
+                if (x < w && (f < bv || (f == bv && lr))) { bv = f; bi = x; }
+            }
+    }
+    auto better = [&](float v2, int i2, float v1, int i1) {
+        if (i2 < 0) return false;
+        if (i1 < 0) return true;
+        if (v2 < v1) return true;
+        if (v2 > v1) return false;
+        return lr ? (i2 > i1) : (i2 < i1);
+    };
+    for (int o = 32; o > 0; o >>= 1) {
+        const float v2 = __shfl_xor(bv, o);
+        const int i2 = __shfl_xor(bi, o);
+        if (better(v2, i2, bv, bi)) { bv = v2; bi = i2; }
+    }
+    if ((tid & 63) == 0) { s_val[tid >> 6] = bv; s_idx[tid >> 6] = bi; }
+    __syncthreads();
+    bv = s_val[0]; bi = s_idx[0];
+#pragma unroll
+    for (int k = 1; k < VPATH_THREADS / 64; k++) if (better(s_val[k], s_idx[k], bv, bi)) { bv = s_val[k]; bi = s_idx[k]; }
+    const float lim = 536870912.0f;
+    const bool ok = (bi >= 0) && (bv < lim || (bv == lim && lr));
+    return ok ? bi : -1;
+}
+
+constexpr int vp1_rows(int delta) { return delta == 1 ? 28 : delta == 2 ? 12 : delta == 3 ? 8 : 4; }
+#define VP1_AHEAD 3
+template <int r>
+__device__ __forceinline__ void vp1_step(const int e, int &o, int &path)
+{
+    asm volatile("v_writelane_b32 %0, %1, %2" : "+v"(path) : "s"(o), "n"(r));
+    o += __builtin_amdgcn_readlane(e, o);
+}
+template <int N, int... Rs>
+__device__ __forceinline__ void vp1_chase(const int (&e)[N], int &o, int &path, std::integer_sequence<int, Rs...>)
+{
+    (vp1_step<Rs>(e[Rs], o, path), ...);
+}
diff --git a/gimp-lqr-plugin_amd/csrc/vpath1_walk.inc b/gimp-lqr-plugin_amd/csrc/vpath1_walk.inc
--- /dev/null
+++ b/gimp-lqr-plugin_amd/csrc/vpath1_walk.inc
@@ -0,0 +1,49 @@
+    constexpr int R = VP1_ROWS, NB = VP1_AHEAD + 1, RL = VP1_ROWS / 4;
+    static_assert(VP1_ROWS % 4 == 0 && VP1_ROWS * DELTA <= 28 && VP1_AHEAD * VP1_ROWS * DELTA + 32 <= 120, "window margin");
+    u32x4 regs[NB][RL];
+    int xa[NB];
+    auto window_base = [&](int cx) { return (cx - 120) & ~15; };
+    auto load_chunk = [&](int b, int y_top, int cx) {
+        const int base = window_base(cx);
+        xa[b] = base;
+        const int voff = min(max(base + 16 * (lane & 15), 0), stride - 16);
+        const int rsub = (lane >> 4) * stride;
+#pragma unroll
+        for (int q = 0; q < RL; q++) {
+            const int row = max((y_top - 4 * q) * stride - rsub, stride);
+            regs[b][q] = *(const GLOBAL_AS u32x4 *) (c.least + (unsigned) (row + voff));
+        }
+    };
+    auto run_chunk = [&](int b, int y_top) {
+        const int relbase = x - 32 - xa[b];
+        int e[R];
+#pragma unroll
+        for (int q = 0; q < RL; q++) *(u32x4 *) (s_win + q * 1024 + lane * 16) = regs[b][q];
+        __builtin_amdgcn_wave_barrier();
+#pragma unroll
+        for (int r = 0; r < R; r++) e[r] = s_win[r * 256 + relbase + lane];
+        int e2[R / 2];
+#pragma unroll
+        for (int k = 0; k < R / 2; k++) e2[k] = e[2 * k] + __builtin_amdgcn_ds_bpermute((lane + e[2 * k]) << 2, e[2 * k + 1]);
+        int o = 32, path = 0;
+        vp1_chase<R / 2>(e2, o, path, std::make_integer_sequence<int, R / 2>{});
+        const int odd = path + s_win[min(lane, R / 2 - 1) * 512 + relbase + path];
+        __builtin_amdgcn_wave_barrier();
+        const int pe = path + x - 32, po = odd + x - 32;
+        const int nrows = min(R, y_top);
+        VP1_RECORD(y_top, nrows, pe, po);
+        x = (nrows == R) ? x + o - 32 : __builtin_amdgcn_readlane((nrows & 1) ? po : pe, nrows >> 1);
+    };
+    int y_top = h - 1;
+#pragma unroll
+    for (int k = 0; k < VP1_AHEAD; k++) load_chunk(k, y_top - k * R, x);
+    while (true) {
+#pragma unroll
+        for (int k = 0; k < NB; k++) {
+            load_chunk((k + VP1_AHEAD) % NB, y_top - VP1_AHEAD * R, x);
+            run_chunk(k, y_top);
+            y_top -= R;
+            if (y_top < 1) break;
+        }
+        if (y_top < 1) break;
+    }
diff --git a/gimp-lqr-plugin_amd/host/lqr_carver.c b/gimp-lqr-plugin_amd/host/lqr_carver.c
--- a/gimp-lqr-plugin_amd/host/lqr_carver.c
+++ b/gimp-lqr-plugin_amd/host/lqr_carver.c
@@ -103,6 +103,7 @@
 
     float *dbg_en, *dbg_m;
     int *dbg_least, dbg_w, dbg_h;
+    int dbg_org, dbg_org_prev, dbg_side;
 };
 
 static const int k_depth_bytes[4] = {1, 2, 4, 8};
@@ -693,6 +694,7 @@
     r->dbg_least = (int *) malloc(n * sizeof(int));
     if (!r->dbg_en || !r->dbg_m || !r->dbg_least) return LQR_NOMEM;
     HIP_CATCH(lqrhip_read_working(r->dev, r->geo.w, r->geo.h, r->dbg_en, r->dbg_m, r->dbg_least));
+    HIP_CATCH(lqrhip_read_seam_flags(r->dev, &r->dbg_org, &r->dbg_org_prev, &r->dbg_side));
     return LQR_OK;
 }
 
@@ -1235,6 +1237,13 @@
     HIP_CATCH(lqrhip_read_working(r->dev, r->geo.w, r->geo.h, en, m, least_dx));
     return LQR_OK;
 }
+int lqrhip_debug_seam_flags(const void *carver, int *org, int *org_prev, int *side)
+{
+    const LqrCarver *r = (const LqrCarver *) carver;
+    if (!r || !r->dbg_m) return LQRHIP_EARG;
+    *org = r->dbg_org; *org_prev = r->dbg_org_prev; *side = r->dbg_side;
+    return 0;
+}
 gint lqrx_carver_debug_width(LqrCarver *r) { return r->dbg_w; }
 gint lqrx_carver_debug_height(LqrCarver *r) { return r->dbg_h; }
 LqrRetVal lqrx_carver_debug_snapshot(LqrCarver *r, gfloat *en, gfloat *m, gint *least_dx)
diff --git a/include/lqr_hip.h b/include/lqr_hip.h
--- a/include/lqr_hip.h
+++ b/include/lqr_hip.h
@@ -110,6 +110,8 @@
 void lqrhip_pool_trim(void);
 int lqrhip_read_vmap(LqrHipCarver *c, int w0, int h0, int w, int level, int depth, int *out);
 int lqrhip_read_working(LqrHipCarver *c, int w, int h, float *en, float *m, int *least_dx);
+int lqrhip_read_seam_flags(LqrHipCarver *c, int *org, int *org_prev, int *side);
+int lqrhip_debug_seam_flags(const void *carver, int *org, int *org_prev, int *side);
 
 void lqrhip_prof_enable(int on);
 void lqrhip_set_update_mode(int mode);
@@ -117,6 +119,8 @@
 void lqrhip_set_carve_fused(int max_images);
 void lqrhip_set_carve_beside(int mode);
 unsigned long long lqrhip_carve_beside_launches(int reset);
+void lqrhip_set_backtrack_beside(int mode);
+unsigned long long lqrhip_backtrack_beside_launches(int reset);
 void lqrhip_set_vpath_mode(int mode, int par_max);
 void lqrhip_set_dp_persistent_limit(int workgroups);
 void lqrhip_set_dp_persistent_px(int px);
```

Measured after the change: 580,300 Mseams*px/s (median of 6 runs). 1.07x the previous value.
